# ExaScience/elprep

Measured on AMD Instinct MI355X. Metric: Mreads/s through sort+markdup+BQSR, 150bp PE, higher is better.
Workload: dtype u8/int32/int64 (integer path; float64 finalize on host)

## Files before the change

elprep_amd/csrc/adapt.hip:

```cpp
#include <cstdlib>

#include "apply_rec.hpp"
#include "common.hpp"
#include "flat.hpp"
#include "sort_plan.hpp"

namespace elp {

__global__ __launch_bounds__(256) void k_adapt_fixed(uint64_t n, const int32_t *__restrict__ pos, const int32_t *__restrict__ refid,
                                                     const uint16_t *__restrict__ flag, const uint64_t *__restrict__ cigar_off,
                                                     const uint32_t *__restrict__ cigar, int32_t *__restrict__ upos, int32_t *__restrict__ score,
                                                     uint64_t *__restrict__ key, uint32_t n_ref, int pos_bits,
                                                     const uint8_t *__restrict__ has_sr) {
  uint64_t i = (uint64_t)blockIdx.x * blockDim.x + threadIdx.x;
  if (i >= n) return;
  const uint16_t f = flag[i];
  const int32_t p = pos[i];
  const int32_t r = refid[i];
  const uint64_t ru = has_sr[i] ? (uint64_t)n_ref + 1 : (r < 0 ? (uint64_t)n_ref : (uint64_t)(uint32_t)r);
  key[i] = (ru << (pos_bits + 1)) | ((uint64_t)(uint32_t)p << 1) | ((f & F_REVERSED) ? 1ull : 0ull);
  int32_t up = 0;
  if ((f & (F_UNMAPPED | F_SECONDARY | F_SUPPLEMENTARY)) == 0) {
    const uint64_t c0 = cigar_off[i], c1 = cigar_off[i + 1];
    up = p;
    if (c1 > c0) {
      if (f & F_REVERSED) {
        int32_t clipped = 1;
        up--;
        for (uint64_t k = c1; k-- > c0;) {
          const uint32_t c = cigar[k];
          const uint32_t op = c & 0xF;
          const int32_t isclip = (op == OP_S || op == OP_H) ? 1 : 0;
          const int32_t isref = op_consumes_ref(op) ? 1 : 0;
          clipped *= isclip;
          up += (isref | clipped) * (int32_t)(c >> 4);
        }
      } else {
        for (uint64_t k = c0; k < c1; k++) {
          const uint32_t c = cigar[k];
          const uint32_t op = c & 0xF;
          if (!(op == OP_S || op == OP_H)) break;
          up -= (int32_t)(c >> 4);
        }
      }
    }
  }
  upos[i] = up;
  score[i] = 0;
}

__device__ __forceinline__ uint32_t first_bytes32(int n) { return n <= 0 ? 0u : (n >= 4 ? 0xFFFFFFFFu : (0xFFFFFFFFu >> (32 - 8 * n))); }

struct ScoreBody {
  static constexpr int NT = FL_THREADS, TILES = 4, RMAX = 1024;
  static constexpr bool TILE_ENDS = false;
  const uint16_t *__restrict__ flag;
  const uint8_t *__restrict__ qual;
  int32_t *score;
  uint64_t *qbounds;
  int32_t *acc;
  uint32_t *lo;
  uint32_t *hi;
  uint8_t *cand;
  const uint4 *mask;
  uint32_t bad;

  __device__ __forceinline__ void stage(uint32_t g0, uint32_t ng) {
    for (uint32_t k = threadIdx.x; k < ng; k += NT) {
      acc[k] = 0;
      lo[k] = 0xFFFFFFFFu;
      hi[k] = 0u;
      cand[k] = (flag[g0 + k] & (F_UNMAPPED | F_SECONDARY | F_SUPPLEMENTARY)) == 0;
    }
  }
  static __device__ __forceinline__ uint32_t part(uint32_t x, uint32_t s) {
    const uint32_t ge15 = ((x + 0x71717171u) & 0x80808080u) >> 7;
    return __builtin_amdgcn_sad_u8(x & (ge15 * 0xFFu), 0u, s);
  }
  static __device__ __forceinline__ uint32_t gt2(uint32_t x) { return (((x | 0x80808080u) - 0x03030303u) | x) & 0x80808080u; }
  static __device__ __forceinline__ uint32_t ge94(uint32_t x) { return x | (x + 0x22222222u); }
  struct Pre { Chunk ch; uint32_t rl; int nb; int k0; };
  __device__ __forceinline__ bool prefetch(uint32_t rl, int k0, int nb, uint64_t qpos, uint32_t, Pre &p) {
    p.rl = rl; p.nb = nb; p.k0 = k0;
    p.ch.load(qual + qpos);
    return true;
  }
  __device__ __forceinline__ void process(Pre &p) {
    const uint4 mk = mask[p.nb];
    const uint32_t x0 = p.ch.w0 & mk.x, x1 = p.ch.w1 & mk.y, x2 = p.ch.w2 & mk.z, x3 = p.ch.w3 & mk.w;
    const uint64_t glo = (uint64_t)gt2(x0) | ((uint64_t)gt2(x1) << 32);
    const uint64_t ghi = (uint64_t)gt2(x2) | ((uint64_t)gt2(x3) << 32);
    if (glo | ghi) {
      const int first = glo ? (__builtin_ctzll(glo) >> 3) : 8 + (__builtin_ctzll(ghi) >> 3);
      const int last = ghi ? 8 + ((63 - __builtin_clzll(ghi)) >> 3) : ((63 - __builtin_clzll(glo)) >> 3);
      atomicMin(&lo[p.rl], (uint32_t)(p.k0 + first));
      atomicMax(&hi[p.rl], (uint32_t)(p.k0 + last + 1));
    }
    if (!cand[p.rl]) return;
    bad |= (ge94(x0) | ge94(x1) | ge94(x2) | ge94(x3)) & 0x80808080u;
    const uint32_t s = part(x3, part(x2, part(x1, part(x0, 0u))));
    if (s) atomicAdd(&acc[p.rl], (int32_t)s);
  }
  __device__ __forceinline__ void group_end(uint32_t g0, uint32_t ng) {
    for (uint32_t k = threadIdx.x; k < ng; k += NT) {
      score[g0 + k] = acc[k];
      qbounds[g0 + k] = (uint64_t)hi[k] | ((uint64_t)lo[k] << 32);
    }
  }
  __device__ __forceinline__ void slots(uint32_t) {}
  __device__ __forceinline__ void retire() {}
  __device__ __forceinline__ void tile_end(uint32_t, uint64_t) {}
};

__global__ __launch_bounds__(FL_THREADS) void k_score_flat(uint64_t n, const uint64_t *__restrict__ qual_off, const uint8_t *__restrict__ qual,
                                                           uint64_t qual_bytes, const uint32_t *__restrict__ tile_first,
                                                           const uint16_t *__restrict__ flag, int32_t *score, uint64_t *qbounds, uint32_t *err) {
  __shared__ FlatLds<ScoreBody::RMAX> L;
  __shared__ int32_t acc[ScoreBody::RMAX];
  __shared__ uint32_t lo[ScoreBody::RMAX], hi[ScoreBody::RMAX];
  __shared__ uint8_t cand[ScoreBody::RMAX];
  __shared__ uint4 mask[17];
  if (threadIdx.x <= 16) {
    const int nb = (int)threadIdx.x;
    mask[nb] = make_uint4(first_bytes32(nb), first_bytes32(nb - 4), first_bytes32(nb - 8), first_bytes32(nb - 12));
  }
  __syncthreads();
  ScoreBody B{flag, qual, score, qbounds, acc, lo, hi, cand, mask, 0u};
  flat_run(qual_off, n, qual_bytes, tile_first, L, B);
  if (__any(B.bad != 0) && (threadIdx.x & 63) == 0) atomicOr(&err[0], 1u);
}

constexpr int SU_WAVES = 8, SU_MAX_LEN = 250;
__device__ __forceinline__ uint32_t su_gt2(uint32_t x) { return (((x | 0x80808080u) - 0x03030303u) | x) & 0x80808080u; }
template <int R>
__global__ __launch_bounds__(64 * SU_WAVES) void k_score_uniform(uint64_t n, uint32_t L, const uint8_t *__restrict__ qual, const uint16_t *__restrict__ flag,
                                                                 int32_t *__restrict__ score, uint64_t *__restrict__ qbounds, uint32_t *err,
                                                                 uint32_t qstride ,
                                                                 unsigned long long *qmask, const uint16_t *__restrict__ rgid, const uint16_t *__restrict__ rg_cov,
                                                                 uint2 *__restrict__ arecs ) {
  extern __shared__ __attribute__((aligned(16))) uint32_t su_lds[];
  const uint32_t lane = threadIdx.x & 63u, wave = threadIdx.x >> 6;
  const uint32_t tile_bytes = 64u * L, tile_words = tile_bytes / 4u + 4u;
  uint32_t *tile = su_lds + (size_t)wave * tile_words;
  const uint32_t s = lane * L, w0 = s >> 2, skip = s & 3u;
  const uint32_t nw = (skip + L + 3u) >> 2, tail = (skip + L) & 3u;
  const uint32_t m_first = 0xFFFFFFFFu << (8u * skip), m_last = tail ? 0xFFFFFFFFu >> (32u - 8u * tail) : 0xFFFFFFFFu;
  uint32_t bad = 0;
  uint32_t qm[3] = {0, 0, 0};
  const uint64_t ngroups = (n + 63) / 64;
  for (uint64_t g = (uint64_t)blockIdx.x * SU_WAVES + wave; g < ngroups; g += (uint64_t)gridDim.x * SU_WAVES) {
    const uint64_t r0 = g * 64;
    const uint8_t *base = qual + r0 * L;
    const uint64_t have = (n - r0 < 64 ? n - r0 : 64) * (uint64_t)L;
    uint4 v[R];
#pragma unroll
    for (int k = 0; k < R; k++) {
      const uint32_t off = (uint32_t)k * 1024u + lane * 16u;
      v[k] = make_uint4(0u, 0u, 0u, 0u);
      if (off < have) v[k] = *reinterpret_cast<const uint4 *>(base + off);
    }
#pragma unroll
    for (int k = 0; k < R; k++) {
      const uint32_t off = (uint32_t)k * 1024u + lane * 16u;
      if (off < tile_bytes) *reinterpret_cast<uint4 *>(tile + off / 4u) = v[k];
    }
    const uint64_t r = r0 + lane;
    if (r < n) {
      const uint16_t f = flag[r];
      const bool cand = (f & (F_UNMAPPED | F_SECONDARY | F_SUPPLEMENTARY)) == 0;
      const uint16_t rg = arecs ? rgid[r] : (uint16_t)ELP_NIL16;
      const uint32_t *rw = tile + w0;
      uint32_t x = rw[0] & m_first;
      if (nw == 1) x &= m_last;
      constexpr uint32_t NONE = 0xFFFFFFFFu;
      uint32_t sum = ScoreBody::part(x, 0u), orx = x;
      uint32_t kf = su_gt2(x) ? 0u : NONE, kl = 0u;
#pragma unroll 8
      for (uint32_t k = 1; k + 1 < nw; k++) {
        x = rw[k];
        sum = ScoreBody::part(x, sum);
        orx |= x;
        const bool gk = su_gt2(x) != 0u;
        kf = min(kf, gk ? k : NONE);
        kl = gk ? k : kl;
      }
      if (nw > 1) {
        x = rw[nw - 1] & m_last;
        sum = ScoreBody::part(x, sum);
        orx |= x;
        const bool gk = su_gt2(x) != 0u;
        kf = min(kf, gk ? nw - 1 : NONE);
        kl = gk ? nw - 1 : kl;
      }
      uint32_t bd = ScoreBody::ge94(orx) & 0x80808080u;
      if (bd) {
        bd = 0;
        for (uint32_t k = 0; k < nw; k++) {
          uint32_t xw = rw[k];
          if (k == 0) xw &= m_first;
          if (k == nw - 1) xw &= m_last;
          bd |= ScoreBody::ge94(xw);
        }
      }
      uint32_t lo = 0xFFFFFFFFu, hi = 0u;
      if (kf != NONE) {
        uint32_t xf = rw[kf], xl = rw[kl];
        if (kf == 0) xf &= m_first;
        if (kf == nw - 1) xf &= m_last;
        if (kl == 0) xl &= m_first;
        if (kl == nw - 1) xl &= m_last;
        lo = kf * 4u + ((uint32_t)__builtin_ctz(su_gt2(xf)) >> 3) - skip;
        hi = kl * 4u + ((31u - (uint32_t)__builtin_clz(su_gt2(xl))) >> 3) - skip + 1u;
      }
      score[r] = cand ? (int32_t)sum : 0;
      qbounds[r] = (uint64_t)hi | ((uint64_t)lo << 32);
      if (cand) bad |= bd & 0x80808080u;
      if (arecs) arecs[r] = rg == ELP_NIL16 ? make_uint2(AR_NO_RG, 0u) : apply_record(L, (int)L, f, (uint64_t)hi | ((uint64_t)lo << 32), rg_cov[rg]);
      if ((uint32_t)g % qstride == 0) {
        for (uint32_t k = 0; k < nw; k++) {
          const uint32_t vm = (k == 0 ? m_first : 0xFFFFFFFFu) & (k + 1 == nw ? m_last : 0xFFFFFFFFu), xw = rw[k];
#pragma unroll
          for (int b = 0; b < 4; b++) {
            const uint32_t q = (xw >> (8 * b)) & 0xFFu, bit = ((vm >> (8 * b)) & 1u) << (q & 31u), ws = q >> 5;
            qm[0] |= ws == 0 ? bit : 0u;
            qm[1] |= ws == 1 ? bit : 0u;
            qm[2] |= ws == 2 ? bit : 0u;
          }
        }
      }
    }
  }
  if (__any(bad != 0) && lane == 0) atomicOr(&err[0], 1u);
  if (__any((qm[0] | qm[1] | qm[2]) != 0)) {
    for (int d = 32; d >= 1; d >>= 1) {
      qm[0] |= __shfl_xor(qm[0], d, 64);
      qm[1] |= __shfl_xor(qm[1], d, 64);
      qm[2] |= __shfl_xor(qm[2], d, 64);
    }
    if (lane == 0) {
      const unsigned long long lo = (unsigned long long)qm[0] | ((unsigned long long)qm[1] << 32);
      if (lo) atomicOr(&qmask[0], lo);
      if (qm[2]) atomicOr(&qmask[1], (unsigned long long)qm[2]);
    }
  }
}
static bool score_uniform_ok(uint32_t L) {
  if (L < 16 || L > (uint32_t)SU_MAX_LEN) return false;
  if (L % 4u) return true;
  return ((L / 4u) % 4u) != 0;
}
template <int R>
static int score_uniform_launch(elp_ctx *c) {
  const uint32_t L = c->uniform_len;
  const size_t dyn = (size_t)SU_WAVES * ((size_t)64 * L + 16);
  const unsigned per_cu = (unsigned)std::max<size_t>(1, (160 * 1024) / (dyn + 256));
  const uint64_t ngroups = (c->n + 63) / 64;
  const unsigned grid = (unsigned)std::min<uint64_t>((ngroups + SU_WAVES - 1) / SU_WAVES, (uint64_t)c->n_cu * per_cu);
  ELP_HIP(c, hipFuncSetAttribute(reinterpret_cast<const void *>(&k_score_uniform<R>), hipFuncAttributeMaxDynamicSharedMemorySize, (int)dyn));
  uint2 *arecs = nullptr;
  if (L >= 16 && L <= 0x7FFF && c->n_rg > 0) {
    ELP_TRY(ensure(c, c->apply_recs, c->n + 4));
    arecs = c->apply_recs.p;
  }
  const uint32_t qstride = (uint32_t)std::min<uint64_t>(128, std::max<uint64_t>(1, ngroups / 8192));
  ELP_LAUNCH(c, "adapt_score", k_score_uniform<R>, dim3(grid), dim3(64 * SU_WAVES), dyn, c->n, L, (const uint8_t *)c->qual.p, (const uint16_t *)c->flag.p,
             c->score.p, c->qbounds.p, c->adapt_err.p, qstride, reinterpret_cast<unsigned long long *>(c->adapt_err.p + 2), (const uint16_t *)c->rgid.p,
             (const uint16_t *)c->rg_cov.p, arecs);
  c->derived.adapt_sampled = true;
  c->derived.apply_recs_valid = arecs != nullptr;
  c->apply_recs_lmax = (int)L;
  return 0;
}
static int score_uniform(elp_ctx *c) {
  switch ((c->uniform_len + 15u) / 16u) {
#define ELP_SU(R) case R: return score_uniform_launch<R>(c);
    ELP_SU(1) ELP_SU(2) ELP_SU(3) ELP_SU(4) ELP_SU(5) ELP_SU(6) ELP_SU(7) ELP_SU(8) ELP_SU(9) ELP_SU(10) ELP_SU(11) ELP_SU(12) ELP_SU(13) ELP_SU(14)
    ELP_SU(15) ELP_SU(16)
#undef ELP_SU
  }
  return set_error(c, ELP_ERR_ARG, "score_uniform: read length %u", c->uniform_len);
}

__global__ __launch_bounds__(256) void k_qual_present_sample(const uint8_t *__restrict__ qual, uint64_t qual_bytes, uint64_t stride, uint64_t span,
                                                             unsigned long long *qmask) {
  const uint64_t ntiles = (qual_bytes + FL_TILE - 1) / FL_TILE;
  uint32_t m[3] = {0, 0, 0};
  for (uint64_t t = (uint64_t)blockIdx.x * stride; t < ntiles; t += (uint64_t)gridDim.x * stride) {
    const uint64_t tb = t * FL_TILE, te = (tb + span < qual_bytes) ? tb + span : qual_bytes;
    for (uint64_t p = tb + (uint64_t)threadIdx.x * 16; p < te; p += 256 * 16) {
      Chunk ch;
      ch.load(qual + p);
      const int nv = (int)((te - p) < 16 ? (te - p) : 16);
#pragma unroll
      for (int i = 0; i < 16; i++) {
        const uint32_t wv = (i >> 2) == 0 ? ch.w0 : ((i >> 2) == 1 ? ch.w1 : ((i >> 2) == 2 ? ch.w2 : ch.w3));
        const uint32_t q = (wv >> (8 * (i & 3))) & 0xFFu;
        const uint32_t bit = (i < nv) ? (1u << (q & 31u)) : 0u;
        const uint32_t wsel = q >> 5;
        m[0] |= wsel == 0 ? bit : 0u;
        m[1] |= wsel == 1 ? bit : 0u;
        m[2] |= wsel == 2 ? bit : 0u;
      }
    }
  }
  for (int d = 32; d >= 1; d >>= 1) {
    m[0] |= __shfl_xor(m[0], d, 64);
    m[1] |= __shfl_xor(m[1], d, 64);
    m[2] |= __shfl_xor(m[2], d, 64);
  }
  if ((threadIdx.x & 63) == 0) {
    const unsigned long long lo = (unsigned long long)m[0] | ((unsigned long long)m[1] << 32);
    if (lo) atomicOr(&qmask[0], lo);
    if (m[2]) atomicOr(&qmask[1], (unsigned long long)m[2]);
  }
}

__global__ __launch_bounds__(256) void k_flat_index(const uint64_t *__restrict__ qual_off, uint64_t n_reads, uint64_t ntiles,
                                                    uint32_t *__restrict__ tile_first) {
  const uint64_t t = (uint64_t)blockIdx.x * blockDim.x + threadIdx.x;
  if (t > ntiles) return;
  if (t == ntiles) { tile_first[t] = (uint32_t)n_reads; return; }
  const uint64_t x = t * FL_TILE;
  uint64_t lo = 0, hi = n_reads;
  while (lo < hi) {
    const uint64_t mid = lo + (hi - lo) / 2;
    if (qual_off[mid] >= x) hi = mid; else lo = mid + 1;
  }
  tile_first[t] = (uint32_t)lo;
}

int ensure_flat_index(elp_ctx *c) {
  if (c->derived.has_flat_index(c->n, c->qual_bytes)) return 0;
  const uint64_t ntiles = (c->qual_bytes + FL_TILE - 1) / FL_TILE;
  ELP_TRY(ensure(c, c->tile_first, ntiles + 2));
  if (c->n)
    ELP_LAUNCH(c, "flat_index", k_flat_index, dim3(blocks_for(ntiles + 1, 256)), dim3(256), 0, (const uint64_t *)c->qual_off.p, c->n, ntiles,
               c->tile_first.p);
  c->derived.flat_index_n = c->n;
  c->derived.flat_index_bytes = c->qual_bytes;
  return 0;
}

__global__ __launch_bounds__(256) void k_uniform_check(uint64_t n, const uint64_t *__restrict__ qual_off, const uint64_t *__restrict__ seq_off,
                                                       const uint32_t *__restrict__ l_seq, uint64_t len, uint64_t sb, uint64_t seq_front, uint32_t *bad) {
  const uint64_t i = (uint64_t)blockIdx.x * blockDim.x + threadIdx.x;
  bool b = false;
  if (i < n) b = qual_off[i] != i * len || seq_off[i] != seq_front + i * sb || (uint64_t)l_seq[i] != len;
  if (i == n) b = qual_off[n] != n * len || seq_off[n] != seq_front + n * sb;
  if (__any(b) && (threadIdx.x & 63) == 0) atomicOr(bad, 1u);
}
int ensure_uniform_len(elp_ctx *c) {
  if (c->derived.has_uniform(c->n, c->qual_bytes)) return 0;
  c->uniform_len = 0;
  c->derived.uniform_n = c->n;
  c->derived.uniform_bytes = c->qual_bytes;
  if (!c->n || c->qual_bytes % c->n) return 0;
  const uint64_t len = c->qual_bytes / c->n;
  if (len == 0 || len > 0x3FFFFFull) return 0;
  uint32_t *bad = c->err_flag.p + 2;
  ELP_HIP(c, hipMemsetAsync(bad, 0, 4, c->stream));
  ELP_LAUNCH(c, "uniform_check", k_uniform_check, dim3(blocks_for(c->n + 1, 256)), dim3(256), 0, c->n, (const uint64_t *)c->qual_off.p,
             (const uint64_t *)c->seq_off.p, (const uint32_t *)c->l_seq.p, len, (len + 1) / 2, (uint64_t)elp_ctx::SEQ_FRONT, bad);
  uint32_t hb = 0;
  ELP_HIP(c, hipMemcpyAsync(&hb, bad, 4, hipMemcpyDeviceToHost, c->stream));
  ELP_HIP(c, elp::stream_wait(c->stream));
  ELP_HIP(c, hipMemsetAsync(bad, 0, 4, c->stream));
  if (!hb) c->uniform_len = (uint32_t)len;
  return 0;
}

int adapt_quality_error(elp_ctx *c) {
  return set_error(c, ELP_ERR_DATA, "Invalid QUAL character (phred > 93) in a duplicate-marking candidate (reference: log.Panic, filters/mark-duplicates.go:64-66)");
}

static int adapt_resolve(elp_ctx *c) {
  if (!c->derived.adapt_pending) return 0;
  uint32_t w[ADAPT_WORDS];
  ELP_HIP(c, hipMemcpyAsync(w, c->adapt_err.p, sizeof w, hipMemcpyDeviceToHost, c->stream));
  ELP_HIP(c, elp::stream_wait(c->stream));
  adapt_note(c, w);
  return 0;
}
void adapt_note(elp_ctx *c, const uint32_t *words) {
  c->derived.adapt_word_read((words[0] & 1u) != 0);
  if (c->derived.adapt_sampled) {
    c->adapt_qmask[0] = (unsigned long long)words[2] | ((unsigned long long)words[3] << 32);
    c->adapt_qmask[1] = (unsigned long long)words[4] | ((unsigned long long)words[5] << 32);
  }
}
int adapt_begin(elp_ctx *c, int *pos_bits_out) {
  ELP_HIP(c, hipSetDevice(c->device));
  const uint64_t n = c->n;
  ELP_TRY(ensure_flat_index(c));
  ELP_TRY(ensure(c, c->upos, n + 1));
  ELP_TRY(ensure(c, c->score, n + 1));
  ELP_TRY(ensure(c, c->key, n + 1));
  ELP_TRY(ensure(c, c->qbounds, n + 1));
  ELP_TRY(ensure(c, c->adapt_err, ADAPT_WORDS + 2));
  ELP_HIP(c, hipMemsetAsync(c->adapt_err.p, 0, ADAPT_WORDS * sizeof(uint32_t), c->stream));
  c->derived.adapt_begins();
  const KeyWidth kw = key_width(c->max_pos, c->n_ref);
  c->key_bits = kw.key_bits;
  *pos_bits_out = kw.pos_bits;
  return 0;
}
int adapt_scores(elp_ctx *c) {
  const uint64_t n = c->n;
  if (!n) return 0;
  if (!c->qual_bytes) {
    ELP_HIP(c, hipMemsetAsync(c->qbounds.p, 0, n * sizeof(uint64_t), c->stream));
    ELP_HIP(c, hipMemsetAsync(c->score.p, 0, n * sizeof(int32_t), c->stream));
    return 0;
  }
  ELP_TRY(ensure_uniform_len(c));
  if (c->uniform_len && score_uniform_ok(c->uniform_len) && c->tune.score_kernel != 1) {
    ELP_TRY(score_uniform(c));
  } else {
    ELP_HIP(c, hipMemsetAsync(c->score.p, 0, n * sizeof(int32_t), c->stream));
    const unsigned grid = (unsigned)std::min<uint64_t>(flat_steps<ScoreBody>(c->qual_bytes), (uint64_t)c->n_cu * 4);
    ELP_LAUNCH(c, "adapt_score_flat", k_score_flat, dim3(grid), dim3(FL_THREADS), 0, n, (const uint64_t *)c->qual_off.p, (const uint8_t *)c->qual.p,
               c->qual_bytes, (const uint32_t *)c->tile_first.p, (const uint16_t *)c->flag.p, c->score.p, c->qbounds.p, c->adapt_err.p);
  }
  c->derived.adapt_pending = true;
  return 0;
}
int ensure_adapted(elp_ctx *c, bool check_quals) {
  if (c->derived.adapted()) {
    if (check_quals) ELP_TRY(adapt_resolve(c));
    return (check_quals && c->derived.adapt_bad_qual) ? adapt_quality_error(c) : 0;
  }
  int pos_bits = 1;
  ELP_TRY(adapt_begin(c, &pos_bits));
  const uint64_t n = c->n;
  if (n) {
    ELP_LAUNCH(c, "adapt_fixed", k_adapt_fixed, dim3(blocks_for(n, 256)), dim3(256), 0, n, (const int32_t *)c->pos.p, (const int32_t *)c->refid.p,
               (const uint16_t *)c->flag.p, (const uint64_t *)c->cigar_off.p, (const uint32_t *)c->cigar.p, c->upos.p, c->score.p, c->key.p,
               (uint32_t)c->n_ref, pos_bits, (const uint8_t *)c->has_sr.p);
    ELP_TRY(adapt_scores(c));
  }
  c->derived.keys = c->derived.scores = true;
  if (check_quals) ELP_TRY(adapt_resolve(c));
  return (check_quals && c->derived.adapt_bad_qual) ? adapt_quality_error(c) : 0;
}
int ensure_keys(elp_ctx *c) { return c->derived.keys ? 0 : ensure_adapted(c, false); }

int ensure_qual_present(elp_ctx *c, bool exact) {
  if (c->derived.have_qual_present) return 0;
  c->qual_present[0] = c->qual_present[1] = 0;
  if (!exact && c->tune.qual_hint != 1 && c->derived.scores && c->derived.adapt_sampled) {
    ELP_TRY(adapt_resolve(c));
    c->qual_present[0] = c->adapt_qmask[0];
    c->qual_present[1] = c->adapt_qmask[1];
  } else if (c->qual_bytes && (exact || c->tune.qual_hint != 1)) {
    unsigned long long *qm;
    ELP_TRY(scratch(c, 6, 4, &qm));
    ELP_HIP(c, hipMemsetAsync(qm, 0, 16, c->stream));
    const uint64_t ntiles = (c->qual_bytes + FL_TILE - 1) / FL_TILE;
    const uint64_t stride = exact ? 1 : std::min<uint64_t>(16, std::max<uint64_t>(1, ntiles / 2048));
    const unsigned grid = (unsigned)std::min<uint64_t>((ntiles + stride - 1) / stride, 2048);
    ELP_LAUNCH(c, "qual_present_sample", k_qual_present_sample, dim3(grid), dim3(256), 0, (const uint8_t *)c->qual.p, c->qual_bytes, stride,
               (exact || stride == 1) ? FL_TILE : (uint64_t)4096, qm);
    ELP_HIP(c, hipMemcpyAsync(c->qual_present, qm, 16, hipMemcpyDeviceToHost, c->stream));
    ELP_HIP(c, elp::stream_wait(c->stream));
  }
  if (!exact && c->tune.qual_hint_drop >= 0) {
    const int q = c->tune.qual_hint_drop;
    if (q < 64) c->qual_present[0] &= ~(1ull << q);
    else if (q < 128) c->qual_present[1] &= ~(1ull << (q - 64));
  }
  c->derived.have_qual_present = true;
  return 0;
}

}
```

elprep_amd/csrc/common.hpp:

```cpp
#pragma once

#include <hip/hip_runtime.h>

#include <sched.h>

#include <cstdarg>
#include <cstdint>
#include <cstdio>
#include <cstring>
#include <map>
#include <mutex>
#include <string>
#include <vector>

#include "../../include/elprep_hip.h"
#include "../../include/elprep_hip_debug.h"
#include "apply_plan.hpp"
#include "derived.hpp"

namespace elp {

constexpr int WAVE = 64;

enum : uint16_t {
  F_MULTIPLE = 0x1, F_PROPER = 0x2, F_UNMAPPED = 0x4, F_NEXT_UNMAPPED = 0x8, F_REVERSED = 0x10, F_NEXT_REVERSED = 0x20,
  F_FIRST = 0x40, F_LAST = 0x80, F_SECONDARY = 0x100, F_QCFAILED = 0x200, F_DUPLICATE = 0x400, F_SUPPLEMENTARY = 0x800
};

enum : uint32_t { OP_M = 0, OP_I = 1, OP_D = 2, OP_N = 3, OP_S = 4, OP_H = 5, OP_P = 6, OP_EQ = 7, OP_X = 8 };

__host__ __device__ inline bool op_consumes_read(uint32_t op) { return op == OP_M || op == OP_I || op == OP_S || op == OP_EQ || op == OP_X; }
__host__ __device__ inline bool op_consumes_ref(uint32_t op) { return op == OP_M || op == OP_D || op == OP_N || op == OP_EQ || op == OP_X; }

size_t debug_guard_bytes();
void debug_guard_arm(void *p, size_t payload_bytes);
void debug_guard_release(void *p);
int debug_guard_check_all();

template <class T>
struct DVec {
  T *p = nullptr;
  size_t cap = 0;
  DVec() = default;
  DVec(const DVec &) = delete;
  DVec &operator=(const DVec &) = delete;
  ~DVec() { release(); }
  void release() {
    if (p) { debug_guard_release(p); (void)hipFree(p); }
    p = nullptr;
    cap = 0;
  }
  size_t bytes() const { return cap * sizeof(T); }
};

struct ProfPending {
  int name_id;
  hipEvent_t a, b;
};

}

struct elp_ctx {
  int device = 0;
  int n_cu = 256;
  hipStream_t stream = nullptr;
  std::string err;
  std::mutex stage_mu;

  bool have_header = false;
  int32_t n_ref = 0, n_rg = 0, n_lib = 0, n_cov = 0;
  std::vector<int32_t> h_ref_len;
  std::vector<uint16_t> h_rg_lib, h_rg_cov;
  elp::DVec<int32_t> ref_len;
  elp::DVec<uint16_t> rg_lib, rg_cov;
  bool dict_replaced = false;
  int32_t n_ref0 = 0;
  std::vector<int32_t> h_ref_len0;

  static constexpr uint64_t SEQ_FRONT = 16;
  uint64_t n = 0, qname_bytes = 0, cigar_ops = 0, seq_bytes = SEQ_FRONT, qual_bytes = 0;
  uint64_t n_sr = 0;
  uint64_t n_filtered = 0;
  elp::DVec<int32_t> refid, pos, next_refid, pnext, tlen;
  elp::DVec<uint16_t> flag, rgid, split;
  elp::DVec<uint8_t> mapq, has_sr;
  elp::DVec<uint32_t> l_seq;
  elp::DVec<uint64_t> qname_off, cigar_off, seq_off, qual_off;
  elp::DVec<uint8_t> qname, seq4, qual;
  elp::DVec<uint32_t> cigar;
  elp::DVec<uint64_t> stage_tmp;
  uint32_t max_qname_len = 0, max_l_seq = 0;
  uint32_t max_split = 0;
  uint32_t max_pos = 0;
  int key_bits = 64;

  elp::Derived derived;
  bool radix_check_pending = false;
  elp::DVec<uint32_t> adapt_err;
  unsigned long long adapt_qmask[2] = {0, 0};
  elp::DVec<uint2> apply_recs;
  int apply_recs_lmax = 0;
  unsigned long long qual_present[2] = {0, 0};
  elp::DVec<int32_t> upos, score;
  elp::DVec<uint64_t> qbounds;
  elp::DVec<uint64_t> key;
  elp::DVec<uint32_t> perm;
  elp::DVec<uint32_t> err_flag;
  elp::DVec<uint32_t> tile_first;
  void *h_pinned = nullptr;
  size_t h_pinned_cap = 0;
  elp::DVec<unsigned long long> radix_state;
  elp::DVec<uint32_t> radix_ticket;
  elp::DVec<unsigned long long> radix_hist;
  elp::DVec<uint32_t> scan_pool;
  elp::DVec<unsigned long long> xchg_hdr;
  elp::DVec<uint32_t> tie_live;
  elp::DVec<uint32_t> md_ctr;
  static constexpr uint32_t MAX_QNAME = 1000;
  static constexpr uint32_t TIE_LIVE_WORDS = 32;
  uint32_t radix_epoch = 0;
  uint32_t uniform_len = 0;

  elp::DVec<uint32_t> mate;
  elp::DVec<uint32_t> pair_win;

  std::vector<uint8_t *> h_ref_seq;
  std::vector<int64_t> h_ref_seq_len;
  std::vector<int32_t *> h_sites;
  std::vector<int64_t> h_n_sites;
  std::vector<uint8_t> ref_flags_dirty;
  std::vector<uint32_t *> h_site_idx;
  elp::DVec<uint8_t *> d_ref_seq;
  elp::DVec<int64_t> d_ref_seq_len;
  elp::DVec<int32_t *> d_sites;
  elp::DVec<uint32_t *> d_site_idx;
  elp::DVec<int64_t> d_n_sites;
  bool bqsr_ptrs_dirty = true;

  static constexpr size_t TABLES_TAIL = 4096;
  elp::DVec<unsigned long long> dev_tables;
  size_t tables_n = 0;
  int tables_max_cycle = 0;
  unsigned long long tables_quals[2] = {0, 0};
  elp::DVec<unsigned long long> tables_pack;
  elp::DVec<uint8_t> lut_rows_dev;
  void *comm = nullptr;
  bool comm_borrowed = false;
  int (*xport)(void *, int64_t *, size_t) = nullptr;
  void *xport_user = nullptr;
  int (*p2p)(void *, int, const void *, size_t, int, void *, size_t) = nullptr;
  void *p2p_user = nullptr;
  int group_rank = 0, group_world = 1;
  elp_ctx *group_owner = nullptr;
  std::vector<elp_ctx *> group_borrowers;

  elp::DVec<uint8_t> raw;
  elp::DVec<uint64_t> raw_off;
  uint64_t raw_n = 0, raw_bytes = 0;
  uint64_t max_raw_rec = 0;
  elp::DVec<uint8_t> rg_ids;
  elp::DVec<uint32_t> rg_ids_off;
  bool have_rg_ids = false;
  elp::DVec<uint8_t> ref_names;
  elp::DVec<uint32_t> ref_names_off;
  std::string h_ref_names;
  std::vector<uint32_t> h_ref_names_off;
  uint32_t max_ref_name = 0;
  bool have_ref_names = false;
  elp::DVec<uint32_t> ref_name_slots;
  uint32_t ref_name_mask = 0;
  bool have_ref_name_table = false;
  static constexpr size_t TAG_WORDS = 65536 / 32;
  bool tag_filter = false;
  std::vector<uint32_t> h_tag_drop;
  elp::DVec<uint32_t> tag_drop;
  bool replace_rg = false;
  std::string replace_rg_id;
  elp::DVec<uint8_t> replace_rg_dev;
  hipStream_t copy_stream = nullptr;
  elp::DVec<uint8_t> lut_dev;
  void *lut_pinned = nullptr;
  size_t lut_pinned_cap = 0;
  hipEvent_t lut_ev = nullptr;
  hipEvent_t apply_ev = nullptr;
  int lut_uploaded_cycle = 0;
  elp::DVec<uint32_t> lut_wk;
  elp::LutDictBuilt dict_built;
  hipEvent_t tables_ev = nullptr;
  void *bounce[2] = {nullptr, nullptr};
  hipEvent_t bounce_ev[2] = {nullptr, nullptr};

  uint32_t *mail = nullptr;
  hipEvent_t mail_ev = nullptr;

  elp_ctx *side[2] = {nullptr, nullptr};
  hipEvent_t side_ev[2] = {nullptr, nullptr};
  hipEvent_t side_done[2] = {nullptr, nullptr};
  bool sort_ahead = false;
  uint64_t presort_n = 0;
  uint64_t *presort_ks = nullptr;
  int presort_idx_bits = 0;

  elp::DVec<uint16_t> snap_flag;
  elp::DVec<uint8_t> snap_qual;
  uint64_t snap_n = 0, snap_qual_bytes = 0;

  struct Tuning {
    int count_kernel = 0;
    int apply_kernel = 0;
    int count3_rlog = -1;
    int qual_hint = 0;
    int qual_hint_drop = -1;
    int pair_table_slots = 1 << 20;
    long long bgzf_piece = 1ll << 30;
    int bgzf_weak_guess = 0;
    int score_kernel = 0;
    int mate_path = 0;
    int radix_tile = 0;
    int sort_pairs = 0;
    int tie_rounds = 0;
    int exchange_piece = 0;
    int emit_pass = 0;
    int sam_pass = 0;
    long long bgzf_inflate_piece = 2ll << 30;
    int bgzf_copy_chunk = 0;
    int bgzf_tok_lds = 0;
    int bgzf_first_chunk_div = 4;
    int bgzf_fixed = 0;
    int bgzf_tok_fail_above = 0;
    int bgzf_stored = 0;
    int apply_wgs = 0;
    int count3_grid = 0;
    int presort_tile = 0;
    int side_priority = 0;
  } tune;

  elp::DVec<uint8_t> scratch[8];

  bool profiling = false;
  const char *prof_prefix = nullptr;
  std::vector<std::string> prof_names;
  std::map<std::string, int> prof_index;
  std::vector<uint64_t> prof_launches;
  std::vector<double> prof_ms;
  std::vector<elp::ProfPending> prof_pending;
};

namespace elp {

class LaneViews {
  struct Item { void *vec; void (*take_back)(void *); };
  std::vector<Item> items;

 public:
  template <class... Col>
  LaneViews(elp_ctx *shadow, elp_ctx *ctx, Col... cols) { (view(shadow->*cols, ctx->*cols), ...); }
  LaneViews(const LaneViews &) = delete;
  LaneViews &operator=(const LaneViews &) = delete;
  ~LaneViews() {
    for (const Item &it : items) it.take_back(it.vec);
  }
  template <class T>
  void view(DVec<T> &to, const DVec<T> &from, bool with_cap = false) {
    to.p = from.p;
    to.cap = with_cap ? from.cap : 0;
    items.push_back(Item{&to, [](void *v) { DVec<T> *d = static_cast<DVec<T> *>(v); d->p = nullptr; d->cap = 0; }});
  }
};

int set_error(elp_ctx *c, int code, const char *fmt, ...);
int prof_begin(elp_ctx *c, const char *name);
void prof_end(elp_ctx *c, int pending);
int prof_flush(elp_ctx *c);
struct ProfScope {
  elp_ctx *c;
  const char *saved;
  ProfScope(elp_ctx *ctx, const char *prefix) : c(ctx), saved(ctx->prof_prefix) { ctx->prof_prefix = prefix; }
  ~ProfScope() { c->prof_prefix = saved; }
};

#define ELP_HIP(ctx, call)                                                                             \
  do {                                                                                                 \
    hipError_t e__ = (call);                                                                           \
    if (e__ != hipSuccess)                                                                             \
      return elp::set_error((ctx), e__ == hipErrorOutOfMemory ? ELP_ERR_NOMEM : ELP_ERR_HIP, "%s failed: %s (%s:%d)", #call, \
                            hipGetErrorString(e__), __FILE__, __LINE__);                               \
  } while (0)

#define ELP_TRY(expr)            \
  do {                           \
    int rc__ = (expr);           \
    if (rc__ != 0) return rc__;  \
  } while (0)

bool sync_spin();
inline void spin_relax(unsigned &spins) {
  if (++spins < 4096u) {
#if defined(__x86_64__) || defined(__i386__)
    __builtin_ia32_pause();
#elif defined(__aarch64__)
    asm volatile("yield");
#endif
  } else {
    sched_yield();
  }
}
inline hipError_t stream_wait(hipStream_t st) {
  if (!sync_spin()) return hipStreamSynchronize(st);
  hipError_t e;
  unsigned spins = 0;
  while ((e = hipStreamQuery(st)) == hipErrorNotReady) spin_relax(spins);
  return e;
}
inline hipError_t event_wait(hipEvent_t ev) {
  if (!sync_spin()) return hipEventSynchronize(ev);
  hipError_t e;
  unsigned spins = 0;
  while ((e = hipEventQuery(ev)) == hipErrorNotReady) spin_relax(spins);
  return e;
}

int debug_poison();
bool debug_trace();

template <class T>
int ensure(elp_ctx *c, DVec<T> &v, size_t n, bool keep = false, size_t keep_elems = 0) {
  if (n <= v.cap) return 0;
  size_t ncap = keep ? (n + n / 2 + 16) : n;
  T *np = nullptr;
  ELP_HIP(c, hipMalloc((void **)&np, ncap * sizeof(T) + debug_guard_bytes()));
  if (debug_guard_bytes()) debug_guard_arm(np, ncap * sizeof(T));
  if (const int pz = debug_poison(); pz >= 0) {
    ELP_HIP(c, hipMemsetAsync(np, pz, ncap * sizeof(T), c->stream));
    ELP_HIP(c, elp::stream_wait(c->stream));
  }
  if (keep && v.p && keep_elems) {
    hipError_t e = hipMemcpyAsync(np, v.p, keep_elems * sizeof(T), hipMemcpyDeviceToDevice, c->stream);
    if (e == hipSuccess) e = elp::stream_wait(c->stream);
    if (e != hipSuccess) {
      (void)hipFree(np);
      return set_error(c, ELP_ERR_HIP, "device copy failed while growing a column: %s", hipGetErrorString(e));
    }
  }
  if (v.p) {
    (void)elp::stream_wait(c->stream);
    debug_guard_release(v.p);
    if (debug_poison() >= 0) { (void)hipMemsetAsync(v.p, 0xDD, v.cap * sizeof(T), c->stream); (void)elp::stream_wait(c->stream); }
    (void)hipFree(v.p);
  }
  v.p = np;
  v.cap = ncap;
  return 0;
}

template <class T>
int scratch(elp_ctx *c, int slot, size_t n, T **out) {
  ELP_TRY(ensure(c, c->scratch[slot], n * sizeof(T) + 256));
  *out = reinterpret_cast<T *>(c->scratch[slot].p);
  return 0;
}

#define ELP_LAUNCH(ctx, name, kernel, grid, block, shmem, ...)                              \
  do {                                                                                      \
    int pp__ = (ctx)->profiling ? elp::prof_begin((ctx), (name)) : -1;                      \
    if (elp::debug_trace()) fprintf(stderr, "[elp] %s\n", (name));                          \
    hipLaunchKernelGGL(kernel, grid, block, shmem, (ctx)->stream, __VA_ARGS__);             \
    if (pp__ >= 0) elp::prof_end((ctx), pp__);                                              \
    ELP_HIP((ctx), hipGetLastError());                                                      \
    if (elp::debug_trace()) ELP_HIP((ctx), elp::stream_wait((ctx)->stream));            \
  } while (0)

inline unsigned blocks_for(uint64_t n, unsigned per_block) { return (unsigned)((n + per_block - 1) / per_block); }

__device__ __forceinline__ uint64_t mix64(uint64_t x) {
  x ^= x >> 30; x *= 0xbf58476d1ce4e5b9ull; x ^= x >> 27; x *= 0x94d049bb133111ebull; x ^= x >> 31;
  return x;
}

__device__ __forceinline__ uint64_t load8(const uint8_t *__restrict__ p) {
  uint64_t w;
  __builtin_memcpy(&w, p, 8);
  return w;
}
__device__ __forceinline__ uint64_t low_bytes(uint64_t w, uint32_t nbytes) {
  return nbytes >= 8 ? w : (w & ((1ull << (8 * nbytes)) - 1ull));
}
__device__ inline int qname_cmp(const uint8_t *__restrict__ q, const uint64_t *__restrict__ off, uint32_t a, uint32_t b) {
  const uint64_t oa = off[a], ob = off[b];
  const uint32_t la = (uint32_t)(off[a + 1] - oa), lb = (uint32_t)(off[b + 1] - ob);
  const uint32_t m = la < lb ? la : lb;
  for (uint32_t i = 0; i < m; i += 8) {
    const uint32_t nb = m - i;
    const uint64_t wa = low_bytes(load8(q + oa + i), nb), wb = low_bytes(load8(q + ob + i), nb);
    if (wa != wb) {
      const uint64_t ba = __builtin_bswap64(wa), bb = __builtin_bswap64(wb);
      return ba < bb ? -1 : 1;
    }
  }
  return la < lb ? -1 : (la > lb ? 1 : 0);
}
__device__ inline bool qname_eq(const uint8_t *__restrict__ q, const uint64_t *__restrict__ off, uint32_t a, uint32_t b) {
  const uint64_t oa = off[a], ob = off[b];
  const uint32_t la = (uint32_t)(off[a + 1] - oa), lb = (uint32_t)(off[b + 1] - ob);
  if (la != lb) return false;
  uint64_t diff = 0;
  for (uint32_t i = 0; i < la && diff == 0; i += 32) {
    const uint64_t a0 = load8(q + oa + i), a1 = load8(q + oa + i + 8), a2 = load8(q + oa + i + 16), a3 = load8(q + oa + i + 24);
    const uint64_t b0 = load8(q + ob + i), b1 = load8(q + ob + i + 8), b2 = load8(q + ob + i + 16), b3 = load8(q + ob + i + 24);
    const uint32_t nb = la - i;
    diff |= low_bytes(a0 ^ b0, nb);
    diff |= nb > 8 ? low_bytes(a1 ^ b1, nb - 8) : 0ull;
    diff |= nb > 16 ? low_bytes(a2 ^ b2, nb - 16) : 0ull;
    diff |= nb > 24 ? low_bytes(a3 ^ b3, nb - 24) : 0ull;
  }
  return diff == 0;
}

__host__ __device__ inline uint16_t mod_flag(uint16_t flag) {
  if ((flag & F_MULTIPLE) == 0) flag &= (uint16_t) ~(F_NEXT_UNMAPPED | F_NEXT_REVERSED);
  if (flag & F_UNMAPPED) flag &= (uint16_t)~F_REVERSED;
  if (flag & F_NEXT_UNMAPPED) flag &= (uint16_t)~F_NEXT_REVERSED;
  return flag;
}

inline void commit_rejects(elp_ctx *c, unsigned long long dropped, unsigned long long tagged) {
  c->n_sr += dropped;
  c->n_filtered += dropped + tagged;
}

int radix_sort_pairs(elp_ctx *c, uint64_t *keys, uint32_t *vals, uint64_t *keys_tmp, uint32_t *vals_tmp, uint64_t n,
                     uint64_t **keys_out, uint32_t **vals_out);
int radix_sort_fused(elp_ctx *c, const uint64_t *keycol, uint64_t n, int key_bits, int idx_bits, uint64_t *buf0, uint64_t *buf1, uint64_t **out);
struct RadixBounds {
  uint32_t *start = nullptr, *nend = nullptr;
  uint32_t mask = 0;
  int shift = 0;
};
int radix_sort_pairs_low(elp_ctx *c, uint64_t *keys, uint32_t *vals, uint64_t *keys_tmp, uint32_t *vals_tmp, uint64_t n, int ndigits,
                         uint64_t **keys_out, uint32_t **vals_out, const uint64_t *first_src = nullptr, bool identity_vals = false,
                         const uint32_t *n_dev = nullptr , RadixBounds bnd = RadixBounds{});
int exclusive_scan_u32(elp_ctx *c, const uint32_t *in, uint32_t *out, uint64_t n, uint32_t *total_host );
int ensure_adapted(elp_ctx *c, bool check_quals = true);
int ensure_keys(elp_ctx *c);
int adapt_begin(elp_ctx *c, int *pos_bits);
int adapt_scores(elp_ctx *c);
int mailbox(elp_ctx *c);
int side_lane(elp_ctx *c, int lane, elp_ctx **out);
int side_join(elp_ctx *c, int lane);
int sort_presort(elp_ctx *c);
void prof_merge_side(elp_ctx *c);
constexpr int ADAPT_WORDS = 6;
void adapt_note(elp_ctx *c, const uint32_t *words );
int adapt_quality_error(elp_ctx *c);
int ensure_uniform_len(elp_ctx *c);
int ensure_qual_present(elp_ctx *c, bool exact = false);
int fetch_err(elp_ctx *c, uint32_t *words );
int radix_check(elp_ctx *c);
void group_release(elp_ctx *c);
int group_sendrecv(elp_ctx *c, int send_peer, const void *send_dev, size_t send_bytes, int recv_peer, void *recv_dev, size_t recv_bytes);
int tables_written(elp_ctx *c);
int stage_reserve(elp_ctx *c, uint64_t n, uint64_t qb, uint64_t co, uint64_t sb, uint64_t lb);
constexpr uint32_t MERGE_SECOND = 0x80000000u;
int keep_concat_src(elp_ctx *groups, uint64_t ng, uint64_t ns, uint32_t *g0_dev, uint32_t *src);
int merge_refuses_queryname(elp_ctx *groups, const char *who);
int merge_spread_slots(elp_ctx *groups, elp_ctx *spread, uint64_t **slots_out);
int keep_coordinate_order(elp_ctx *c, uint64_t n_out, uint64_t *keys, uint32_t *bad_dev, bool *in_order);
int stage_recode_seq(elp_ctx *c, uint64_t from, uint64_t bytes);
inline void clear_run_settings(elp_ctx *c) { c->tag_filter = false; c->replace_rg = false; c->replace_rg_id.clear(); }
inline bool same_replace_rg(const elp_ctx *a, const elp_ctx *b) { return a->replace_rg == b->replace_rg && a->replace_rg_id == b->replace_rg_id; }
int install_dictionary(elp_ctx *c, int32_t n_ref, const int32_t *ref_len);
int staging_refused_after_replace(elp_ctx *c, const char *who);
int stage_bam_columns(elp_ctx *c, uint32_t n_rec, uint64_t piece_bytes, uint64_t raw_end, uint64_t max_raw_rec, uint16_t split_id);
int bgzf_frame(elp_ctx *c, const uint8_t *raw, uint64_t n_bytes, uint8_t *out);
int bgzf_deflate(elp_ctx *c, const uint8_t *raw, uint64_t n_bytes, uint8_t *out, uint64_t *out_bytes);

}
```

elprep_amd/csrc/ctx.hip:

```cpp
#include "common.hpp"

namespace elp {

namespace {
constexpr size_t GUARD = 4096;
constexpr uint8_t GUARD_BYTE = 0xC3;
std::mutex guard_mu;
std::map<void *, size_t> guard_of;
int guard_check_one(void *p, size_t payload) {
  uint8_t host[GUARD];
  if (hipDeviceSynchronize() != hipSuccess || hipMemcpy(host, static_cast<uint8_t *>(p) + payload, GUARD, hipMemcpyDeviceToHost) != hipSuccess) return 0;
  for (size_t k = 0; k < GUARD; k++)
    if (host[k] != GUARD_BYTE) {
      fprintf(stderr, "[elp] ELP_DEBUG_GUARD: byte %zu behind the end of a %zu-byte device buffer was overwritten (0x%02x)\n", k, payload, host[k]);
      return 1;
    }
  return 0;
}
}
size_t debug_guard_bytes() {
  static const size_t v = [] { const char *e = getenv("ELP_DEBUG_GUARD"); return (e && *e && *e != '0') ? GUARD : (size_t)0; }();
  return v;
}
void debug_guard_arm(void *p, size_t payload) {
  (void)hipMemset(static_cast<uint8_t *>(p) + payload, GUARD_BYTE, GUARD);
  (void)hipDeviceSynchronize();
  std::lock_guard<std::mutex> lk(guard_mu);
  guard_of[p] = payload;
}
void debug_guard_release(void *p) {
  if (!debug_guard_bytes()) return;
  size_t payload = 0;
  {
    std::lock_guard<std::mutex> lk(guard_mu);
    auto it = guard_of.find(p);
    if (it == guard_of.end()) return;
    payload = it->second;
    guard_of.erase(it);
  }
  if (guard_check_one(p, payload)) abort();
}
int debug_guard_check_all() {
  if (!debug_guard_bytes()) return 0;
  std::lock_guard<std::mutex> lk(guard_mu);
  int bad = 0;
  for (auto &kv : guard_of) bad += guard_check_one(kv.first, kv.second);
  return bad;
}

bool sync_spin() {
  static const bool v = [] { const char *e = getenv("ELP_SYNC_SPIN"); return !(e && *e == '0'); }();
  return v;
}
bool debug_trace() {
  static const bool v = [] { const char *e = getenv("ELP_DEBUG_TRACE"); return e && *e && *e != '0'; }();
  return v;
}
int debug_poison() {
  static const int v = [] {
    const char *e = getenv("ELP_DEBUG_POISON");
    return (e && *e) ? (int)(strtol(e, nullptr, 0) & 0xFF) : -1;
  }();
  return v;
}


int set_error(elp_ctx *c, int code, const char *fmt, ...) {
  char buf[1024];
  va_list ap;
  va_start(ap, fmt);
  vsnprintf(buf, sizeof buf, fmt, ap);
  va_end(ap);
  if (c) c->err = buf;
  return code;
}

int prof_begin(elp_ctx *c, const char *name0) {
  const std::string name = c->prof_prefix ? std::string(c->prof_prefix) + name0 : std::string(name0);
  auto it = c->prof_index.find(name);
  int id;
  if (it == c->prof_index.end()) {
    id = (int)c->prof_names.size();
    c->prof_names.push_back(name);
    c->prof_index[name] = id;
    c->prof_launches.push_back(0);
    c->prof_ms.push_back(0.0);
  } else {
    id = it->second;
  }
  ProfPending p;
  p.name_id = id;
  if (hipEventCreate(&p.a) != hipSuccess) return -1;
  if (hipEventCreate(&p.b) != hipSuccess) { (void)hipEventDestroy(p.a); return -1; }
  (void)hipEventRecord(p.a, c->stream);
  c->prof_pending.push_back(p);
  return (int)c->prof_pending.size() - 1;
}
void prof_end(elp_ctx *c, int pending) { (void)hipEventRecord(c->prof_pending[pending].b, c->stream); }
int prof_flush(elp_ctx *c) {
  if (c->prof_pending.empty()) return 0;
  ELP_HIP(c, elp::stream_wait(c->stream));
  for (auto &p : c->prof_pending) {
    float ms = 0.f;
    if (hipEventElapsedTime(&ms, p.a, p.b) == hipSuccess) {
      c->prof_ms[p.name_id] += ms;
      c->prof_launches[p.name_id] += 1;
    }
    (void)hipEventDestroy(p.a);
    (void)hipEventDestroy(p.b);
  }
  c->prof_pending.clear();
  return 0;
}

__global__ void k_rebase_offsets(const uint64_t *__restrict__ src, uint64_t *__restrict__ dst, uint64_t n_plus_1, uint64_t base,
                                 uint64_t src0) {
  uint64_t i = (uint64_t)blockIdx.x * blockDim.x + threadIdx.x;
  if (i < n_plus_1) dst[i] = src[i] - src0 + base;
}

__device__ __forceinline__ uint32_t recode_byte(uint32_t b) {
  constexpr uint64_t TAB = 0x8888888388828108ull;
  return (uint32_t)((TAB >> (4 * (b >> 4))) & 15u) | ((uint32_t)((TAB >> (4 * (b & 15u))) & 15u) << 4);
}
__global__ __launch_bounds__(256) void k_recode_seq(uint8_t *__restrict__ seq, uint64_t nbytes) {
  const uint64_t i = ((uint64_t)blockIdx.x * blockDim.x + threadIdx.x) * 16;
  if (i >= nbytes) return;
  if (i + 16 <= nbytes) {
    uint32_t w[4];
    __builtin_memcpy(w, seq + i, 16);
#pragma unroll
    for (int k = 0; k < 4; k++) {
      const uint32_t x = w[k];
      w[k] = recode_byte(x & 0xFFu) | (recode_byte((x >> 8) & 0xFFu) << 8) | (recode_byte((x >> 16) & 0xFFu) << 16) | (recode_byte(x >> 24) << 24);
    }
    __builtin_memcpy(seq + i, w, 16);
  } else {
    for (uint64_t k = i; k < nbytes; k++) seq[k] = (uint8_t)recode_byte(seq[k]);
  }
}

int stage_recode_seq(elp_ctx *c, uint64_t from, uint64_t bytes) {
  hipLaunchKernelGGL(k_recode_seq, dim3(blocks_for((bytes + 15) / 16, 256)), dim3(256), 0, c->stream, c->seq4.p + from, bytes);
  ELP_HIP(c, hipGetLastError());
  return 0;
}

int fetch_err(elp_ctx *c, uint32_t *words) {
  ELP_HIP(c, hipMemcpyAsync(words, c->err_flag.p, 4 * sizeof(uint32_t), hipMemcpyDeviceToHost, c->stream));
  ELP_HIP(c, elp::stream_wait(c->stream));
  c->radix_check_pending = false;
  if (words[0] & 256u) {
    const uint32_t w0 = words[0] & ~256u;
    ELP_HIP(c, hipMemcpyAsync(c->err_flag.p, &w0, 4, hipMemcpyHostToDevice, c->stream));
    ELP_HIP(c, elp::stream_wait(c->stream));
    c->derived.radix_timed_out();
    return set_error(c, ELP_ERR_HIP, "radix sort: tile look-back timed out");
  }
  return 0;
}
int mailbox(elp_ctx *c) {
  if (!c->mail) ELP_HIP(c, hipHostMalloc((void **)&c->mail, 1024 * sizeof(uint32_t), hipHostMallocDefault));
  if (!c->mail_ev) ELP_HIP(c, hipEventCreateWithFlags(&c->mail_ev, hipEventDisableTiming));
  return 0;
}
int side_lane(elp_ctx *c, int lane, elp_ctx **out) {
  if (!c->side[lane]) {
    elp_ctx *s = new elp_ctx();
    s->device = c->device;
    s->n_cu = c->n_cu;
    int prio_lo = 0, prio_hi = 0;
    (void)hipDeviceGetStreamPriorityRange(&prio_lo, &prio_hi);
    const hipError_t se = c->tune.side_priority != 1 ? hipStreamCreateWithFlags(&s->stream, hipStreamNonBlocking)
                                                     : hipStreamCreateWithPriority(&s->stream, hipStreamNonBlocking, prio_hi);
    if (se != hipSuccess || ensure(s, s->err_flag, 4) != 0 ||
        hipMemsetAsync(s->err_flag.p, 0, 16, s->stream) != hipSuccess) {
      if (s->stream) (void)hipStreamDestroy(s->stream);
      delete s;
      return set_error(c, ELP_ERR_HIP, "the side lane's stream could not be made");
    }
    c->side[lane] = s;
  }
  if (!c->side_ev[lane]) ELP_HIP(c, hipEventCreateWithFlags(&c->side_ev[lane], hipEventDisableTiming));
  if (!c->side_done[lane]) ELP_HIP(c, hipEventCreateWithFlags(&c->side_done[lane], hipEventDisableTiming));
  ELP_HIP(c, hipEventRecord(c->side_ev[lane], c->stream));
  ELP_HIP(c, hipStreamWaitEvent(c->side[lane]->stream, c->side_ev[lane], 0));
  c->side[lane]->profiling = c->profiling;
  c->side[lane]->tune = c->tune;
  *out = c->side[lane];
  return 0;
}
int side_join(elp_ctx *c, int lane) {
  ELP_HIP(c, hipEventRecord(c->side_done[lane], c->side[lane]->stream));
  ELP_HIP(c, hipStreamWaitEvent(c->stream, c->side_done[lane], 0));
  return 0;
}
void prof_merge_side(elp_ctx *c) {
  for (int lane = 0; lane < 2; lane++) {
    elp_ctx *s = c->side[lane];
    if (!s) continue;
    (void)prof_flush(s);
    for (size_t k = 0; k < s->prof_names.size(); k++) {
      if (!s->prof_launches[k]) continue;
      auto it = c->prof_index.find(s->prof_names[k]);
      int id;
      if (it == c->prof_index.end()) {
        id = (int)c->prof_names.size();
        c->prof_names.push_back(s->prof_names[k]);
        c->prof_index[s->prof_names[k]] = id;
        c->prof_launches.push_back(0);
        c->prof_ms.push_back(0.0);
      } else {
        id = it->second;
      }
      c->prof_launches[id] += s->prof_launches[k];
      c->prof_ms[id] += s->prof_ms[k];
      s->prof_launches[k] = 0;
      s->prof_ms[k] = 0.0;
    }
  }
}
int radix_check(elp_ctx *c) {
  if (!c->radix_check_pending) return 0;
  uint32_t e[4];
  return fetch_err(c, e);
}

int release_bqsr_inputs(elp_ctx *c) {
  ELP_HIP(c, elp::stream_wait(c->stream));
  for (auto &p : c->h_ref_seq) if (p) { (void)hipFree(p); p = nullptr; }
  for (auto &p : c->h_sites) if (p) { (void)hipFree(p); p = nullptr; }
  for (auto &p : c->h_site_idx) if (p) { (void)hipFree(p); p = nullptr; }
  for (auto &v : c->h_ref_seq_len) v = 0;
  for (auto &v : c->h_n_sites) v = 0;
  c->bqsr_ptrs_dirty = true;
  return 0;
}
int install_dictionary(elp_ctx *c, int32_t n_ref, const int32_t *ref_len) {
  ELP_TRY(ensure(c, c->ref_len, (size_t)n_ref + 1));
  ELP_TRY(release_bqsr_inputs(c));
  const std::vector<int32_t> len(ref_len, ref_len + n_ref);
  c->n_ref = n_ref;
  c->h_ref_len = len;
  c->have_ref_names = false;
  c->have_ref_name_table = false;
  if (n_ref) ELP_HIP(c, hipMemcpyAsync(c->ref_len.p, c->h_ref_len.data(), (size_t)n_ref * sizeof(int32_t), hipMemcpyHostToDevice, c->stream));
  ELP_HIP(c, elp::stream_wait(c->stream));
  c->h_ref_seq.assign((size_t)n_ref, nullptr);
  c->h_ref_seq_len.assign((size_t)n_ref, 0);
  c->h_sites.assign((size_t)n_ref, nullptr);
  c->h_site_idx.assign((size_t)n_ref, nullptr);
  c->h_n_sites.assign((size_t)n_ref, 0);
  c->ref_flags_dirty.assign((size_t)n_ref, 0);
  c->bqsr_ptrs_dirty = true;
  return 0;
}
int staging_refused_after_replace(elp_ctx *c, const char *who) {
  return set_error(c, ELP_ERR_ARG, "%s: the reference dictionary was replaced (elp_replace_reference_dictionary): the staged refids are the new "
                   "dictionary's, the header's are the old one's; call elp_reset or elp_set_header first", who);
}

}

using namespace elp;

extern "C" {

int elp_debug_check_guards(void) { return elp::debug_guard_check_all(); }


int elp_create(int device_ordinal, elp_ctx **out) {
  if (!out) return ELP_ERR_ARG;
  *out = nullptr;
  int ndev = 0;
  if (hipGetDeviceCount(&ndev) != hipSuccess || ndev <= 0) return ELP_ERR_HIP;
  if (device_ordinal < 0 || device_ordinal >= ndev) return ELP_ERR_ARG;
  if (hipSetDevice(device_ordinal) != hipSuccess) return ELP_ERR_HIP;
  hipDeviceProp_t prop;
  if (hipGetDeviceProperties(&prop, device_ordinal) != hipSuccess) return ELP_ERR_HIP;
  if (strncmp(prop.gcnArchName, "gfx950", 6) != 0) return ELP_ERR_UNSUPPORTED;
  elp_ctx *c = new elp_ctx();
  c->device = device_ordinal;
  c->n_cu = prop.multiProcessorCount > 0 ? prop.multiProcessorCount : 256;
  if (hipStreamCreateWithFlags(&c->stream, hipStreamNonBlocking) != hipSuccess) { delete c; return ELP_ERR_HIP; }
  if (ensure(c, c->err_flag, 4) != 0 || hipMemsetAsync(c->err_flag.p, 0, 16, c->stream) != hipSuccess) { delete c; return ELP_ERR_HIP; }
  *out = c;
  return ELP_OK;
}

void elp_destroy(elp_ctx *c) {
  if (!c) return;
  (void)hipSetDevice(c->device);
  (void)elp::stream_wait(c->stream);
  for (auto &p : c->prof_pending) { (void)hipEventDestroy(p.a); (void)hipEventDestroy(p.b); }
  if (c->lut_pinned) (void)hipHostFree(c->lut_pinned);
  if (c->lut_ev) (void)hipEventDestroy(c->lut_ev);
  if (c->apply_ev) (void)hipEventDestroy(c->apply_ev);
  for (auto p : c->h_ref_seq) if (p) (void)hipFree(p);
  for (auto p : c->h_sites) if (p) (void)hipFree(p);
  for (auto p : c->h_site_idx) if (p) (void)hipFree(p);
  if (c->h_pinned) (void)hipHostFree(c->h_pinned);
  for (int lane = 0; lane < 2; lane++) {
    if (c->side[lane]) {
      (void)elp::stream_wait(c->side[lane]->stream);
      for (auto &p : c->side[lane]->prof_pending) { (void)hipEventDestroy(p.a); (void)hipEventDestroy(p.b); }
      (void)hipStreamDestroy(c->side[lane]->stream);
      delete c->side[lane];
      c->side[lane] = nullptr;
    }
    if (c->side_ev[lane]) (void)hipEventDestroy(c->side_ev[lane]);
    if (c->side_done[lane]) (void)hipEventDestroy(c->side_done[lane]);
  }
  if (c->mail) (void)hipHostFree(c->mail);
  if (c->mail_ev) (void)hipEventDestroy(c->mail_ev);
  for (int k = 0; k < 2; k++) {
    if (c->bounce[k]) (void)hipHostFree(c->bounce[k]);
    if (c->bounce_ev[k]) (void)hipEventDestroy(c->bounce_ev[k]);
  }
  if (c->copy_stream) (void)hipStreamDestroy(c->copy_stream);
  if (c->tables_ev) (void)hipEventDestroy(c->tables_ev);
  group_release(c);
  (void)hipStreamDestroy(c->stream);
  delete c;
}

const char *elp_last_error(const elp_ctx *c) { return c ? c->err.c_str() : "null context"; }

int elp_sync(elp_ctx *c) {
  if (!c) return ELP_ERR_ARG;
  if (c->radix_check_pending) return radix_check(c);
  ELP_HIP(c, elp::stream_wait(c->stream));
  return 0;
}

void *elp_stream(elp_ctx *c) { return c ? (void *)c->stream : nullptr; }

int elp_set_header(elp_ctx *c, const elp_header *h) {
  if (!c || !h || h->n_ref < 0 || h->n_rg < 0 || (h->n_ref && !h->ref_len) || (h->n_rg && (!h->rg_lib || !h->rg_cov)))
    return set_error(c, ELP_ERR_ARG, "elp_set_header: bad arguments");
  ELP_HIP(c, hipSetDevice(c->device));
  if (c->dict_replaced) ELP_TRY(release_bqsr_inputs(c));
  c->n_ref = h->n_ref; c->n_rg = h->n_rg; c->n_lib = h->n_lib; c->n_cov = h->n_cov;
  c->derived.header_changed();
  clear_run_settings(c);
  c->h_ref_len.assign(h->ref_len, h->ref_len + h->n_ref);
  c->n_ref0 = h->n_ref;
  c->h_ref_len0 = c->h_ref_len;
  c->dict_replaced = false;
  c->have_ref_names = false;
  c->have_ref_name_table = false;
  c->h_rg_lib.assign(h->rg_lib, h->rg_lib + h->n_rg);
  c->h_rg_cov.assign(h->rg_cov, h->rg_cov + h->n_rg);
  for (int i = 0; i < h->n_rg; i++) {
    if (c->h_rg_lib[i] != ELP_NIL16 && c->h_rg_lib[i] >= h->n_lib) return set_error(c, ELP_ERR_ARG, "rg_lib[%d] out of range", i);
    if (c->h_rg_cov[i] >= h->n_cov) return set_error(c, ELP_ERR_ARG, "rg_cov[%d] out of range", i);
  }
  ELP_TRY(ensure(c, c->ref_len, (size_t)h->n_ref + 1));
  ELP_TRY(ensure(c, c->rg_lib, (size_t)h->n_rg + 1));
  ELP_TRY(ensure(c, c->rg_cov, (size_t)h->n_rg + 1));
  if (h->n_ref) ELP_HIP(c, hipMemcpyAsync(c->ref_len.p, h->ref_len, h->n_ref * sizeof(int32_t), hipMemcpyHostToDevice, c->stream));
  if (h->n_rg) {
    ELP_HIP(c, hipMemcpyAsync(c->rg_lib.p, h->rg_lib, h->n_rg * sizeof(uint16_t), hipMemcpyHostToDevice, c->stream));
    ELP_HIP(c, hipMemcpyAsync(c->rg_cov.p, h->rg_cov, h->n_rg * sizeof(uint16_t), hipMemcpyHostToDevice, c->stream));
  }
  ELP_HIP(c, elp::stream_wait(c->stream));
  c->h_ref_seq.resize(h->n_ref, nullptr);
  c->h_ref_seq_len.resize(h->n_ref, 0);
  c->h_sites.resize(h->n_ref, nullptr);
  c->h_site_idx.resize(h->n_ref, nullptr);
  c->h_n_sites.resize(h->n_ref, 0);
  c->ref_flags_dirty.assign(h->n_ref, 0);
  c->bqsr_ptrs_dirty = true;
  c->have_header = true;
  return 0;
}

}
namespace elp {
int stage_reserve(elp_ctx *c, uint64_t n, uint64_t qb, uint64_t co, uint64_t sb, uint64_t lb) {
  bool keep = c->n > 0;
  ELP_TRY(ensure(c, c->refid, n, keep, c->n));
  ELP_TRY(ensure(c, c->pos, n, keep, c->n));
  ELP_TRY(ensure(c, c->next_refid, n, keep, c->n));
  ELP_TRY(ensure(c, c->pnext, n, keep, c->n));
  ELP_TRY(ensure(c, c->tlen, n, keep, c->n));
  ELP_TRY(ensure(c, c->flag, n, keep, c->n));
  ELP_TRY(ensure(c, c->rgid, n, keep, c->n));
  ELP_TRY(ensure(c, c->split, n, keep, c->n));
  ELP_TRY(ensure(c, c->mapq, n, keep, c->n));
  ELP_TRY(ensure(c, c->has_sr, n, keep, c->n));
  ELP_TRY(ensure(c, c->l_seq, n, keep, c->n));
  ELP_TRY(ensure(c, c->qname_off, n + 1, keep, c->n + 1));
  ELP_TRY(ensure(c, c->cigar_off, n + 1, keep, c->n + 1));
  ELP_TRY(ensure(c, c->seq_off, n + 1, keep, c->n + 1));
  ELP_TRY(ensure(c, c->qual_off, n + 1, keep, c->n + 1));
  ELP_TRY(ensure(c, c->qname, qb + 64, keep, c->qname_bytes));
  ELP_TRY(ensure(c, c->cigar, co + 4, keep, c->cigar_ops));
  ELP_TRY(ensure(c, c->seq4, sb + 32, keep, c->seq_bytes));
  ELP_TRY(ensure(c, c->qual, lb + 32, keep, c->qual_bytes));
  return 0;
}
}
extern "C" {

int elp_reserve(elp_ctx *c, uint64_t n, uint64_t qb, uint64_t co, uint64_t sb, uint64_t lb) {
  if (!c) return ELP_ERR_ARG;
  std::lock_guard<std::mutex> g(c->stage_mu);
  ELP_HIP(c, hipSetDevice(c->device));
  return stage_reserve(c, n, qb, co, sb + elp_ctx::SEQ_FRONT, lb);
}

int elp_reset(elp_ctx *c) {
  if (!c) return ELP_ERR_ARG;
  std::lock_guard<std::mutex> g(c->stage_mu);
  c->n = c->qname_bytes = c->cigar_ops = c->qual_bytes = 0;
  c->seq_bytes = elp_ctx::SEQ_FRONT;
  c->n_sr = 0;
  c->n_filtered = 0;
  c->raw_n = c->raw_bytes = 0;
  c->max_raw_rec = 0;
  c->max_split = 0;
  c->max_qname_len = c->max_l_seq = 0;
  c->max_pos = 0;
  c->derived.records_changed();
  clear_run_settings(c);
  if (c->dict_replaced) {
    ELP_HIP(c, hipSetDevice(c->device));
    ELP_TRY(install_dictionary(c, c->n_ref0, c->h_ref_len0.data()));
    c->derived.header_changed();
    c->dict_replaced = false;
  }
  return 0;
}

uint64_t elp_num_records(const elp_ctx *c) { return c ? c->n : 0; }
uint64_t elp_num_sorted(const elp_ctx *c) { return c ? c->n - c->n_sr : 0; }
uint64_t elp_num_qual_bytes(const elp_ctx *c) { return c ? c->qual_bytes : 0; }

int elp_stage(elp_ctx *c, const elp_batch *b) {
  if (!c || !b) return ELP_ERR_ARG;
  std::lock_guard<std::mutex> g(c->stage_mu);
  ELP_HIP(c, hipSetDevice(c->device));
  if (!c->have_header) return set_error(c, ELP_ERR_ARG, "elp_stage: call elp_set_header first");
  if (c->dict_replaced) return staging_refused_after_replace(c, "elp_stage");
  uint64_t n = b->n;
  if (n == 0) return 0;
  if (c->n + n > 0xFFFFFFF0ull) return set_error(c, ELP_ERR_UNSUPPORTED, "more than 2^32-16 records per context");
  uint64_t q0 = b->qname_off[0], c0 = b->cigar_off[0], s0 = b->seq_off[0], l0 = b->qual_off[0];
  uint64_t qb = b->qname_off[n] - q0, co = b->cigar_off[n] - c0, sb = b->seq_off[n] - s0, lb = b->qual_off[n] - l0;
  ELP_TRY(stage_reserve(c, c->n + n, c->qname_bytes + qb, c->cigar_ops + co, c->seq_bytes + sb, c->qual_bytes + lb));
  hipStream_t st = c->stream;
  uint64_t at = c->n;
#define H2D(dst, src, cnt, T) ELP_HIP(c, hipMemcpyAsync((dst), (src), (cnt) * sizeof(T), hipMemcpyHostToDevice, st))
  if (lb) H2D(c->qual.p + c->qual_bytes, b->qual + l0, lb, uint8_t);
  if (sb) {
    H2D(c->seq4.p + c->seq_bytes, b->seq4 + s0, sb, uint8_t);
    hipLaunchKernelGGL(k_recode_seq, dim3(blocks_for((sb + 15) / 16, 256)), dim3(256), 0, st, c->seq4.p + c->seq_bytes, sb);
    ELP_HIP(c, hipGetLastError());
  }
  if (qb) H2D(c->qname.p + c->qname_bytes, b->qname + q0, qb, uint8_t);
  if (co) H2D(c->cigar.p + c->cigar_ops, b->cigar + c0, co, uint32_t);
  H2D(c->refid.p + at, b->refid, n, int32_t);
  H2D(c->pos.p + at, b->pos, n, int32_t);
  H2D(c->next_refid.p + at, b->next_refid, n, int32_t);
  H2D(c->pnext.p + at, b->pnext, n, int32_t);
  H2D(c->tlen.p + at, b->tlen, n, int32_t);
  H2D(c->flag.p + at, b->flag, n, uint16_t);
  H2D(c->rgid.p + at, b->rgid, n, uint16_t);
  if (b->split) H2D(c->split.p + at, b->split, n, uint16_t);
  else ELP_HIP(c, hipMemsetAsync(c->split.p + at, 0, n * sizeof(uint16_t), st));
  H2D(c->mapq.p + at, b->mapq, n, uint8_t);
  H2D(c->l_seq.p + at, b->l_seq, n, uint32_t);
  if (b->has_sr) H2D(c->has_sr.p + at, b->has_sr, n, uint8_t);
  else ELP_HIP(c, hipMemsetAsync(c->has_sr.p + at, 0, n, st));
  ELP_TRY(ensure(c, c->stage_tmp, 4 * (n + 1)));
  unsigned blk = 256, grd = blocks_for(n + 1, blk);
  struct { const uint64_t *src; uint64_t *dst; uint64_t base; } offs[4] = {
      {b->qname_off, c->qname_off.p + at, c->qname_bytes}, {b->cigar_off, c->cigar_off.p + at, c->cigar_ops},
      {b->seq_off, c->seq_off.p + at, c->seq_bytes}, {b->qual_off, c->qual_off.p + at, c->qual_bytes}};
  for (int k = 0; k < 4; k++) H2D(c->stage_tmp.p + (size_t)k * (n + 1), offs[k].src, n + 1, uint64_t);
  for (int k = 0; k < 4; k++) {
    hipLaunchKernelGGL(k_rebase_offsets, dim3(grd), dim3(blk), 0, st, (const uint64_t *)(c->stage_tmp.p + (size_t)k * (n + 1)), offs[k].dst, n + 1, offs[k].base,
                       offs[k].src[0]);
    ELP_HIP(c, hipGetLastError());
  }
#undef H2D
  uint64_t n_sr = 0;
  uint32_t max_split = c->max_split;
  uint32_t max_qname_len = c->max_qname_len, max_l_seq = c->max_l_seq, max_pos = c->max_pos;
  int scan_rc = 0;
  for (uint64_t i = 0; i < n && !scan_rc; i++) {
    uint64_t ql = b->qname_off[i + 1] - b->qname_off[i];
    if (ql > elp_ctx::MAX_QNAME) scan_rc = set_error(c, ELP_ERR_UNSUPPORTED, "record %llu: QNAME of %llu bytes (limit %u)", (unsigned long long)i, (unsigned long long)ql, elp_ctx::MAX_QNAME);
    if (b->has_sr && b->has_sr[i]) n_sr++;
    if (b->split && b->split[i] > max_split) max_split = b->split[i];
    if (ql > max_qname_len) max_qname_len = (uint32_t)ql;
    if (b->l_seq[i] > max_l_seq) max_l_seq = b->l_seq[i];
    if ((uint32_t)b->pos[i] > max_pos) max_pos = (uint32_t)b->pos[i];
    if (b->qual_off[i + 1] - b->qual_off[i] > 0x3FFFFFull || b->l_seq[i] > 0x3FFFFFu)
      scan_rc = set_error(c, ELP_ERR_UNSUPPORTED, "record %llu: more than 4194303 bases", (unsigned long long)i);
    if (b->rgid[i] != ELP_NIL16 && b->rgid[i] >= c->n_rg) scan_rc = set_error(c, ELP_ERR_ARG, "record %llu: rgid %u not in header", (unsigned long long)i, b->rgid[i]);
    if (b->refid[i] >= c->n_ref) scan_rc = set_error(c, ELP_ERR_ARG, "record %llu: refid %d not in header", (unsigned long long)i, b->refid[i]);
  }
  if (scan_rc) { (void)elp::stream_wait(st); return scan_rc; }
  ELP_HIP(c, elp::stream_wait(st));
  c->n += n; c->qname_bytes += qb; c->cigar_ops += co; c->seq_bytes += sb; c->qual_bytes += lb;
  c->n_sr += n_sr;
  c->max_split = max_split;
  c->max_qname_len = max_qname_len; c->max_l_seq = max_l_seq; c->max_pos = max_pos;
  c->derived.records_changed();
  return 0;
}

int elp_stage_columns(elp_ctx *c, uint64_t n, const int32_t *refid, const int32_t *pos, const int32_t *next_refid, const int32_t *pnext, const int32_t *tlen,
                      const uint16_t *flag, const uint8_t *mapq, const uint16_t *rgid, const uint8_t *has_sr, const uint32_t *l_seq,
                      const uint64_t *qname_off, const uint8_t *qname, const uint64_t *cigar_off, const uint32_t *cigar, const uint64_t *seq_off,
                      const uint8_t *seq4, const uint64_t *qual_off, const uint8_t *qual, const uint16_t *split) {
  if (!c) return ELP_ERR_ARG;
  if (n && (!refid || !pos || !next_refid || !pnext || !tlen || !flag || !mapq || !rgid || !l_seq || !qname_off || !cigar_off || !seq_off || !qual_off))
    return set_error(c, ELP_ERR_ARG, "elp_stage_columns: a required column is NULL");
  elp_batch b;
  b.n = n; b.refid = refid; b.pos = pos; b.next_refid = next_refid; b.pnext = pnext; b.tlen = tlen; b.flag = flag; b.mapq = mapq; b.rgid = rgid;
  b.has_sr = has_sr; b.l_seq = l_seq; b.qname_off = qname_off; b.qname = qname; b.cigar_off = cigar_off; b.cigar = cigar; b.seq_off = seq_off;
  b.seq4 = seq4; b.qual_off = qual_off; b.qual = qual; b.split = split;
  return elp_stage(c, &b);
}

int elp_set_header_columns(elp_ctx *c, int32_t n_ref, const int32_t *ref_len, int32_t n_rg, const uint16_t *rg_lib, const uint16_t *rg_cov, int32_t n_lib,
                           int32_t n_cov) {
  elp_header h;
  h.n_ref = n_ref; h.ref_len = ref_len; h.n_rg = n_rg; h.rg_lib = rg_lib; h.rg_cov = rg_cov; h.n_lib = n_lib; h.n_cov = n_cov;
  return elp_set_header(c, &h);
}

static int d2h(elp_ctx *c, void *dst, const void *src, size_t bytes) {
  if (!bytes) return 0;
  ELP_HIP(c, hipSetDevice(c->device));
  ELP_HIP(c, hipMemcpyAsync(dst, src, bytes, hipMemcpyDeviceToHost, c->stream));
  ELP_HIP(c, elp::stream_wait(c->stream));
  return 0;
}

int elp_get_permutation(elp_ctx *c, uint32_t *out) {
  if (!c || (!out && c->n)) return ELP_ERR_ARG;
  if (!c->derived.sorted) return set_error(c, ELP_ERR_ARG, "elp_get_permutation: call elp_sort_coordinate, elp_sort_queryname or elp_order_keep first");
  ELP_TRY(radix_check(c));
  return d2h(c, out, c->perm.p, c->n * sizeof(uint32_t));
}
int elp_get_flags(elp_ctx *c, uint16_t *out) {
  if (!c || (!out && c->n)) return ELP_ERR_ARG;
  ELP_TRY(radix_check(c));
  return d2h(c, out, c->flag.p, c->n * sizeof(uint16_t));
}
int elp_get_adapted(elp_ctx *c, int32_t *upos, int32_t *score) {
  if (!c) return ELP_ERR_ARG;
  ELP_TRY(ensure_adapted(c));
  if (upos) ELP_TRY(d2h(c, upos, c->upos.p, c->n * sizeof(int32_t)));
  if (score) ELP_TRY(d2h(c, score, c->score.p, c->n * sizeof(int32_t)));
  return 0;
}
int elp_get_qual(elp_ctx *c, uint8_t *out) {
  if (!c || (!out && c->qual_bytes)) return ELP_ERR_ARG;
  return d2h(c, out, c->qual.p, c->qual_bytes);
}

int elp_snapshot(elp_ctx *c) {
  if (!c) return ELP_ERR_ARG;
  ELP_HIP(c, hipSetDevice(c->device));
  ELP_TRY(ensure(c, c->snap_flag, c->n + 1));
  ELP_TRY(ensure(c, c->snap_qual, c->qual_bytes + 16));
  if (c->n) ELP_HIP(c, hipMemcpyAsync(c->snap_flag.p, c->flag.p, c->n * sizeof(uint16_t), hipMemcpyDeviceToDevice, c->stream));
  if (c->qual_bytes) ELP_HIP(c, hipMemcpyAsync(c->snap_qual.p, c->qual.p, c->qual_bytes, hipMemcpyDeviceToDevice, c->stream));
  c->snap_n = c->n;
  c->snap_qual_bytes = c->qual_bytes;
  c->derived.have_snapshot = true;
  return 0;
}
int elp_rollback(elp_ctx *c) {
  if (!c) return ELP_ERR_ARG;
  if (!c->derived.have_snapshot || c->snap_n != c->n || c->snap_qual_bytes != c->qual_bytes)
    return set_error(c, ELP_ERR_ARG, "elp_rollback: no snapshot of the current record set");
  ELP_HIP(c, hipSetDevice(c->device));
  if (c->n) ELP_HIP(c, hipMemcpyAsync(c->flag.p, c->snap_flag.p, c->n * sizeof(uint16_t), hipMemcpyDeviceToDevice, c->stream));
  if (c->qual_bytes) ELP_HIP(c, hipMemcpyAsync(c->qual.p, c->snap_qual.p, c->qual_bytes, hipMemcpyDeviceToDevice, c->stream));
  c->derived.flag_qual_restored();
  return 0;
}

int elp_set_tuning(elp_ctx *c, const char *key, int64_t value) {
  if (!c || !key) return ELP_ERR_ARG;
  const std::string k(key);
  const int v = (int)value;
  if (k == "count_kernel") c->tune.count_kernel = v;
  else if (k == "apply_kernel") c->tune.apply_kernel = v;
  else if (k == "bgzf_piece") { if (value < 1) return set_error(c, ELP_ERR_ARG, "elp_set_tuning: bgzf_piece must be positive"); c->tune.bgzf_piece = value; }
  else if (k == "bgzf_weak_guess") c->tune.bgzf_weak_guess = v;
  else if (k == "score_kernel") { c->tune.score_kernel = v; c->derived.score_tuning_changed(); }
  else if (k == "count3_rlog") c->tune.count3_rlog = v;
  else if (k == "qual_hint") { c->tune.qual_hint = v; c->derived.hint_tuning_changed(); }
  else if (k == "qual_hint_drop") { c->tune.qual_hint_drop = v; c->derived.hint_tuning_changed(); }
  else if (k == "pair_table_slots") {
    if (v == 0) { c->tune.pair_table_slots = 1 << 20; return 0; }
    if (v < 2 || v > (1 << 20) || (v & (v - 1))) return set_error(c, ELP_ERR_ARG, "elp_set_tuning: pair_table_slots must be a power of two >= 2");
    c->tune.pair_table_slots = v;
  } else if (k == "mate_path") {
    if (value != 0 && value != 2) return set_error(c, ELP_ERR_ARG, "elp_set_tuning: mate_path is 0 (the library decides) or 2 (every candidate through the table)");
    c->tune.mate_path = v;
  } else if (k == "tie_rounds") c->tune.tie_rounds = v;
  else if (k == "radix_tile") c->tune.radix_tile = v;
  else if (k == "sort_pairs") c->tune.sort_pairs = v;
  else if (k == "exchange_piece") c->tune.exchange_piece = v;
  else if (k == "emit_pass") c->tune.emit_pass = v;
  else if (k == "sam_pass") c->tune.sam_pass = v;
  else if (k == "bgzf_stored") c->tune.bgzf_stored = v;
  else if (k == "bgzf_tok_fail_above") c->tune.bgzf_tok_fail_above = v;
  else if (k == "bgzf_fixed") c->tune.bgzf_fixed = v;
  else if (k == "bgzf_first_chunk_div") c->tune.bgzf_first_chunk_div = v;
  else if (k == "bgzf_tok_lds") c->tune.bgzf_tok_lds = v;
  else if (k == "bgzf_copy_chunk") c->tune.bgzf_copy_chunk = v;
  else if (k == "bgzf_inflate_piece") { if (value < 1) return set_error(c, ELP_ERR_ARG, "elp_set_tuning: bgzf_inflate_piece must be positive"); c->tune.bgzf_inflate_piece = value; }
  else if (k == "md_fused" || k == "bgzf_inflate") {
    if (value != 0) return set_error(c, ELP_ERR_ARG, "elp_set_tuning: key '%s' is retired (only 0 is accepted)", key);
  } else if (k == "apply_wgs") c->tune.apply_wgs = v;
  else if (k == "presort_tile") c->tune.presort_tile = v;
  else if (k == "count3_grid") { if (value < 0) return set_error(c, ELP_ERR_ARG, "elp_set_tuning: count3_grid must not be negative"); c->tune.count3_grid = v; }
  else if (k == "side_priority") c->tune.side_priority = v;
  else return set_error(c, ELP_ERR_ARG, "elp_set_tuning: unknown key '%s'", key);
  return 0;
}

int elp_profile_enable(elp_ctx *c, int on) {
  if (!c) return ELP_ERR_ARG;
  if (!on) { ELP_TRY(prof_flush(c)); prof_merge_side(c); }
  c->profiling = on != 0;
  for (int lane = 0; lane < 2; lane++)
    if (c->side[lane]) c->side[lane]->profiling = c->profiling;
  return 0;
}
int elp_profile_reset(elp_ctx *c) {
  if (!c) return ELP_ERR_ARG;
  ELP_TRY(prof_flush(c));
  prof_merge_side(c);
  for (auto &v : c->prof_launches) v = 0;
  for (auto &v : c->prof_ms) v = 0.0;
  return 0;
}
int elp_profile_count(elp_ctx *c) {
  if (!c) return ELP_ERR_ARG;
  if (prof_flush(c) != 0) return ELP_ERR_HIP;
  prof_merge_side(c);
  return (int)c->prof_names.size();
}
int elp_profile_get(elp_ctx *c, int index, const char **name, uint64_t *launches, double *total_ms) {
  if (!c || index < 0 || index >= (int)c->prof_names.size()) return ELP_ERR_ARG;
  if (name) *name = c->prof_names[index].c_str();
  if (launches) *launches = c->prof_launches[index];
  if (total_ms) *total_ms = c->prof_ms[index];
  return 0;
}

}
```

elprep_amd/csrc/markdup.hip:

```cpp
#include "common.hpp"
#include "markdup_plan.hpp"

namespace elp {

constexpr uint32_t EMPTY = 0xFFFFFFFFu;
constexpr unsigned long long PB_EMPTY = ~0ull;

struct MdCols {
  uint64_t n;
  const int32_t *refid;
  const uint16_t *flag_in;
  const uint16_t *rgid;
  const uint16_t *rg_lib;
  const uint16_t *split;
  const int32_t *upos, *score;
  const uint64_t *qname_off;
  const uint8_t *qname;
};

__device__ __forceinline__ bool is_candidate(uint16_t f) { return (f & (F_UNMAPPED | F_SECONDARY | F_SUPPLEMENTARY)) == 0; }
__device__ __forceinline__ bool is_true_pair(uint16_t f) { return (f & (F_MULTIPLE | F_NEXT_UNMAPPED)) == F_MULTIPLE; }
__device__ __forceinline__ uint16_t lib_of(const MdCols &m, uint32_t i) {
  const uint16_t rg = m.rgid[i];
  return rg == ELP_NIL16 ? (uint16_t)ELP_NIL16 : m.rg_lib[rg];
}
__device__ __forceinline__ uint32_t ld_agent(const uint32_t *p) { return __hip_atomic_load(p, __ATOMIC_RELAXED, __HIP_MEMORY_SCOPE_AGENT); }
__device__ __forceinline__ unsigned long long ld_agent64(const unsigned long long *p) {
  return __hip_atomic_load(p, __ATOMIC_RELAXED, __HIP_MEMORY_SCOPE_AGENT);
}

__device__ __forceinline__ bool key_eq(const uint4 &a, const uint4 &b) { return a.x == b.x && a.y == b.y && a.z == b.z && a.w == b.w; }
__device__ __forceinline__ uint64_t frag_hash(const uint4 &k) {
  const uint64_t h = ((uint64_t)k.x << 32) | k.y;
  return mix64(mix64(h) ^ (((uint64_t)k.w << 32) | (uint64_t)k.z));
}

template <class Eq>
__device__ __forceinline__ uint32_t find_or_insert(uint32_t *table, uint64_t mask, uint64_t h, uint32_t i, Eq eq, uint64_t limit = ~0ull) {
  uint64_t s = h & mask;
  for (uint64_t probes = 0;; probes++) {
    if (probes > limit) return EMPTY;
    const uint32_t cur = atomicCAS(&table[s], EMPTY, i);
    if (cur == EMPTY) return i;
    if (cur == i || eq(cur, i)) return cur;
    s = (s + 1) & mask;
  }
}

__global__ __launch_bounds__(256) void k_frag_insert(MdCols m, const uint4 *__restrict__ fkey, const uint32_t *__restrict__ flist, uint32_t nf,
                                                     uint32_t *table, uint64_t mask, uint32_t *__restrict__ frep, unsigned long long *fbest) {
  const uint32_t j = blockIdx.x * blockDim.x + threadIdx.x;
  if (j >= nf) return;
  const uint32_t i = flist[j];
  const uint4 mine = fkey[i];
  const uint32_t rep = find_or_insert(table, mask, frag_hash(mine), i, [&](uint32_t a, uint32_t) { return key_eq(fkey[a], mine); });
  frep[i] = rep;
  atomicMax(&fbest[rep], (unsigned long long)(uint32_t)m.score[i]);
}
__global__ __launch_bounds__(256) void k_frag_bits(const uint32_t *__restrict__ table, uint64_t nwords, uint32_t *__restrict__ bits) {
  const uint64_t w = (uint64_t)blockIdx.x * blockDim.x + threadIdx.x;
  if (w >= nwords) return;
  const uint4 *t = reinterpret_cast<const uint4 *>(table + 32 * w);
  uint32_t b = 0;
#pragma unroll
  for (int k = 0; k < 8; k++) {
    const uint4 v = t[k];
    b |= (v.x != EMPTY ? 1u : 0u) << (4 * k) | (v.y != EMPTY ? 2u : 0u) << (4 * k) | (v.z != EMPTY ? 4u : 0u) << (4 * k) | (v.w != EMPTY ? 8u : 0u) << (4 * k);
  }
  bits[w] = b;
}
__device__ __forceinline__ void tournament(const MdCols &m, uint32_t *winner, uint32_t me) {
  uint32_t w = ld_agent(winner);
  for (;;) {
    if (w == EMPTY) {
      const uint32_t old = atomicCAS(winner, EMPTY, me);
      if (old == EMPTY) return;
      w = old;
      continue;
    }
    const int cq = qname_cmp(m.qname, m.qname_off, me, w);
    const bool better = cq < 0 || (cq == 0 && me > w);
    if (!better) return;
    const uint32_t old = atomicCAS(winner, w, me);
    if (old == w) return;
    w = old;
  }
}

__global__ __launch_bounds__(256) void k_frag_tie(MdCols m, const uint32_t *__restrict__ flist, uint32_t nf, const uint32_t *__restrict__ frep,
                                                  const unsigned long long *__restrict__ fbest, uint32_t *fwinner) {
  const uint32_t j = blockIdx.x * blockDim.x + threadIdx.x;
  if (j >= nf) return;
  const uint32_t i = flist[j];
  const uint32_t rep = frep[i];
  const unsigned long long b = fbest[rep];
  if ((b >> 63) || (unsigned long long)(uint32_t)m.score[i] != b) return;
  tournament(m, &fwinner[rep], (uint32_t)i);
}

__global__ __launch_bounds__(256) void k_frag_flag(MdCols m, const uint32_t *__restrict__ flist, uint32_t nf, const uint32_t *__restrict__ frep,
                                                   const unsigned long long *__restrict__ fbest, const uint32_t *__restrict__ fwinner,
                                                   uint16_t *__restrict__ flag_out) {
  const uint32_t j = blockIdx.x * blockDim.x + threadIdx.x;
  if (j >= nf) return;
  const uint32_t i = flist[j];
  const uint32_t rep = frep[i];
  const unsigned long long b = fbest[rep];
  const bool dup = (b >> 63) || (unsigned long long)(uint32_t)m.score[i] < b || fwinner[rep] != (uint32_t)i;
  if (dup) flag_out[i] = (uint16_t)(flag_out[i] | F_DUPLICATE);
}

struct PairKey { uint4 k1, k2; };
__device__ __forceinline__ PairKey pair_key(const uint4 &second, const uint4 &first) {
  const int32_t r1 = (int32_t)second.x, r2 = (int32_t)first.x, p1 = (int32_t)second.y, p2 = (int32_t)first.y;
  const bool v1 = second.z & 1u, v2 = first.z & 1u;
  const bool swap = r1 > r2 || (r1 == r2 && (p1 > p2 || (p1 == p2 && v1 && !v2)));
  return swap ? PairKey{first, second} : PairKey{second, first};
}
__device__ __forceinline__ bool pair_key_eq(const PairKey &a, const PairKey &b) {
  return a.k1.x == b.k1.x && a.k2.x == b.k2.x && a.k1.y == b.k1.y && a.k2.y == b.k2.y && a.k1.z == b.k1.z && ((a.k2.z ^ b.k2.z) & 1u) == 0 &&
         a.k1.w == b.k1.w;
}

__device__ __forceinline__ uint64_t pair_hash(const PairKey &k) {
  uint64_t h = mix64(((uint64_t)k.k1.x << 32) | k.k2.x);
  h = mix64(h ^ (((uint64_t)k.k1.y << 32) | k.k2.y));
  return mix64(h ^ (((uint64_t)k.k1.z << 1) | (k.k2.z & 1u)) ^ ((uint64_t)k.k1.w << 40));
}

__device__ __forceinline__ uint64_t qname_hash(const MdCols &m, uint32_t i) {
  const uint64_t o = m.qname_off[i];
  const uint32_t l = (uint32_t)(m.qname_off[i + 1] - o);
  uint64_t h = 0x9e3779b97f4a7c15ull ^ l;
  for (uint32_t k = 0; k < l; k += 8) h = (h ^ low_bytes(load8(m.qname + o + k), l - k)) * 0xff51afd7ed558ccdull + (h >> 29);
  return mix64(h ^ ((uint64_t)lib_of(m, i) << 48) ^ ((uint64_t)m.split[i] << 24));
}
__device__ __forceinline__ bool mate_key_eq(const MdCols &m, const uint4 *__restrict__ fkey, uint32_t a, const uint4 &kb, uint32_t b) {
  const uint4 ka = fkey[a];
  return (ka.z >> 1) == (kb.z >> 1) && ka.w == kb.w && qname_eq(m.qname, m.qname_off, a, b);
}
__device__ __forceinline__ bool is_mate_candidate(uint16_t f) { return is_candidate(f) && is_true_pair(f); }

enum : uint8_t { MC_NONE = 0, MC_TABLE = 1, MC_LEAD = 2, MC_FOLLOW = 3, MC_KIND = 3, MC_TABBED = 4  };
constexpr uint32_t MATE_BIG = 0xFFFFFFFEu;

__global__ __launch_bounds__(256) void k_bloom_coarse(const uint32_t *__restrict__ bloom, uint32_t n_lines, uint32_t *__restrict__ coarse) {
  const uint32_t line = blockIdx.x * 256 + threadIdx.x;
  bool nz = false;
  if (line < n_lines) {
    const uint4 *l = reinterpret_cast<const uint4 *>(bloom + (size_t)line * 16);
    const uint4 a = l[0], b = l[1], c2 = l[2], d = l[3];
    nz = (a.x | a.y | a.z | a.w | b.x | b.y | b.z | b.w | c2.x | c2.y | c2.z | c2.w | d.x | d.y | d.z | d.w) != 0;
  }
  const unsigned long long bits = __ballot(nz);
  if ((threadIdx.x & 63) == 0 && line < n_lines) {
    coarse[line >> 5] = (uint32_t)bits;
    coarse[(line >> 5) + 1] = (uint32_t)(bits >> 32);
  }
}

__device__ __forceinline__ void mate_table_insert(const MdCols &m, const uint4 *__restrict__ fkey, uint32_t i, uint64_t h, uint32_t *table, uint64_t mask, uint32_t *mate,
                                                  uint32_t *rep_of, uint32_t *err) {
  const uint4 mine = fkey[i];
  const uint32_t rep = find_or_insert(table, mask, h, i, [&](uint32_t a, uint32_t b) { return mate_key_eq(m, fkey, a, mine, b); }, mask);
  if (rep == EMPTY) atomicOr(&err[1], 2u);
  else if (rep != i) {
    rep_of[i] = rep;
    const uint32_t old = atomicCAS(&mate[rep], EMPTY, i);
    if (old == EMPTY) mate[i] = rep;
    else {
      rep_of[rep] = MATE_BIG;
      atomicOr(&err[1], 1u);
    }
  }
}
__global__ __launch_bounds__(256) void k_mate_table(MdCols m, const uint4 *__restrict__ fkey, const uint8_t *__restrict__ code, const uint32_t *__restrict__ hash32,
                                                    const uint32_t *__restrict__ hash_lo, const uint32_t *__restrict__ tab_list, const uint32_t *__restrict__ tab_cnt,
                                                    uint32_t cap, uint32_t *table, uint64_t mask, uint32_t *mate, uint32_t *rep_of, uint32_t *err) {
  __shared__ uint32_t first[65];
  if (threadIdx.x < 64) {
    const uint32_t c = tab_cnt[threadIdx.x * 16u];
    uint32_t incl = c;
    for (int d = 1; d < 64; d <<= 1) {
      const uint32_t up = __shfl_up(incl, d, 64);
      if ((int)threadIdx.x >= d) incl += up;
    }
    first[threadIdx.x + 1] = incl;
    if (threadIdx.x == 0) first[0] = 0;
  }
  __syncthreads();
  for (uint32_t g = blockIdx.x * 256u + threadIdx.x; g < first[64]; g += gridDim.x * 256u) {
    uint32_t lo = 0, hi = 64;
    while (hi - lo > 1) {
      const uint32_t mid = (lo + hi) >> 1;
      if (first[mid] <= g) lo = mid; else hi = mid;
    }
    const uint32_t i = tab_list[(size_t)lo * cap + (g - first[lo])];
    const uint64_t h = (code[i] & MC_KIND) == MC_TABLE ? ((uint64_t)hash32[i] << 32) | hash_lo[i] : qname_hash(m, i);
    mate_table_insert(m, fkey, i, h, table, mask, mate, rep_of, err);
  }
}

__global__ __launch_bounds__(256) void k_mate_pairs(MdCols m, const uint4 *__restrict__ fkey, uint8_t *__restrict__ code,
                                                    const uint32_t *__restrict__ hash32, const uint32_t *__restrict__ hash_lo, const uint32_t *__restrict__ bloom,
                                                    uint32_t bloom_mask, const uint32_t *__restrict__ coarse ,
                                                    uint32_t *table, uint64_t mask, uint32_t *mate, uint32_t *rep_of, uint32_t *err, int fixed,
                                                    uint64_t *__restrict__ pk, uint32_t *__restrict__ pv,
                                                    uint32_t *__restrict__ tab_list , uint32_t *tab_cnt, uint32_t tab_cap) {
  const uint64_t base = (uint64_t)blockIdx.x * (256 * MP_R) + threadIdx.x;
  uint8_t cd[MP_R];
  uint4 mine[MP_R], prev[MP_R];
  uint32_t hi[MP_R], hl[MP_R], bl[MP_R];
  int32_t sc[MP_R];
#pragma unroll
  for (int r = 0; r < MP_R; r++) {
    const uint64_t i = base + (uint64_t)r * 256;
    const bool in = i < m.n;
    cd[r] = in ? (uint8_t)(code[i] & MC_KIND) : (uint8_t)MC_NONE;
    mine[r] = in ? fkey[i] : make_uint4(0, 0, 0, 0);
    const uint32_t h0 = in ? hash32[i] : 0u, h1 = (in && i > 0) ? hash32[i - 1] : 0u;
    hi[r] = cd[r] == MC_LEAD ? h0 : h1;
    hl[r] = (in && cd[r] == MC_TABLE) ? hash_lo[i] : 0u;
  }
#pragma unroll
  for (int r = 0; r < MP_R; r++) {
    const uint64_t i = base + (uint64_t)r * 256;
    const bool cand = cd[r] != MC_NONE;
    bl[r] = ~0u;
    if (cand && cd[r] != MC_TABLE) {
      const uint32_t wi = (hi[r] >> 5) & bloom_mask, line = wi >> 4;
      bl[r] = (coarse && ((coarse[line >> 5] >> (line & 31u)) & 1u)) ? bloom[wi] : 0u;
    }
    const bool fol = cd[r] == MC_FOLLOW;
    prev[r] = fol ? fkey[i - 1] : make_uint4(0, 0, 0, 0);
    sc[r] = fol ? m.score[i] + m.score[i - 1] : 0;
  }
#pragma unroll
  for (int r = 0; r < MP_R; r++) {
    const uint64_t i = base + (uint64_t)r * 256;
    bool own = false, want_tab = false;
    uint64_t key = 0;
    if (cd[r] != MC_NONE) {
      const bool tab = cd[r] == MC_TABLE || ((bl[r] >> (hi[r] & 31u)) & 1u);
      if (!tab) {
        mate[i] = cd[r] == MC_LEAD ? (uint32_t)i + 1 : (uint32_t)i - 1;
        if (cd[r] == MC_FOLLOW) {
          if (fixed) {
            own = true;
            key = ((uint64_t)(uint32_t)sc[r] << 32) | (uint32_t)pair_hash(pair_key(mine[r], prev[r]));
          } else {
            code[i] = (uint8_t)(cd[r] | MC_TABBED);
          }
        }
      } else {
        code[i] = (uint8_t)(cd[r] | MC_TABBED);
        if (tab_list) want_tab = true;
        else mate_table_insert(m, fkey, (uint32_t)i, cd[r] == MC_TABLE ? ((uint64_t)hash32[i] << 32) | hl[r] : qname_hash(m, (uint32_t)i), table, mask, mate, rep_of, err);
      }
    }
    if (tab_list) {
      const unsigned long long tm = __ballot(want_tab);
      if (tm) {
        const int lane = threadIdx.x & 63, leader = __ffsll((long long)tm) - 1;
        const uint32_t li = blockIdx.x & 63u;
        uint32_t at = 0;
        if (lane == leader) at = atomicAdd(&tab_cnt[li * 16u], (uint32_t)__popcll(tm));
        at = __shfl(at, leader, 64) + (uint32_t)__popcll(tm & ((1ull << lane) - 1ull));
        if (want_tab) tab_list[(size_t)li * tab_cap + at] = (uint32_t)i;
      }
    }
    if (fixed) {
      const int next_owns = __shfl_down((int)own, 1, 64);
      if (own) {
        pk[i >> 1] = key;
        pv[i >> 1] = (uint32_t)i;
      } else if (!(threadIdx.x & 1u) && !next_owns && i < m.n) {
        pk[i >> 1] = 0xFFFFFFFF00000000ull | (uint32_t)mix64(i);
        pv[i >> 1] = EMPTY;
      }
    }
  }
}

__global__ __launch_bounds__(256) void k_big_collect(uint64_t n, const uint32_t *__restrict__ rep_of, uint32_t *mate, uint64_t *__restrict__ keys,
                                                     uint32_t *__restrict__ vals, uint32_t *count) {
  const uint64_t i = (uint64_t)blockIdx.x * 256 + threadIdx.x;
  if (i >= n) return;
  const uint32_t r = rep_of[i];
  if (r == EMPTY) return;
  uint32_t rep;
  if (r == MATE_BIG) rep = (uint32_t)i;
  else if (rep_of[r] == MATE_BIG) rep = r;
  else return;
  const uint32_t at = atomicAdd(count, 1u);
  keys[at] = ((uint64_t)rep << 32) | (uint64_t)i;
  vals[at] = (uint32_t)i;
  mate[i] = EMPTY;
}
__global__ __launch_bounds__(256) void k_big_pair(uint32_t cnt, const uint64_t *__restrict__ keys, uint32_t *mate) {
  const uint32_t j = blockIdx.x * 256 + threadIdx.x;
  if (j >= cnt) return;
  const uint32_t rep = (uint32_t)(keys[j] >> 32);
  if (j > 0 && (uint32_t)(keys[j - 1] >> 32) == rep) return;
  for (uint32_t k = j; k + 1 < cnt && (uint32_t)(keys[k + 1] >> 32) == rep; k += 2) {
    const uint32_t a = (uint32_t)keys[k], b = (uint32_t)keys[k + 1];
    mate[a] = b;
    mate[b] = a;
  }
}

__device__ __forceinline__ uint64_t pair_entry(const MdCols &m, const uint4 &later, const uint4 &earlier, uint32_t i, uint32_t mt) {
  return ((uint64_t)(uint32_t)(m.score[i] + m.score[mt]) << 32) | (uint32_t)pair_hash(pair_key(later, earlier));
}
__global__ __launch_bounds__(256) void k_pair_list_table(MdCols m, const uint4 *__restrict__ fkey, const uint32_t *__restrict__ mate,
                                                         const uint8_t *__restrict__ code, uint64_t *__restrict__ pk, uint32_t *__restrict__ pv,
                                                         uint32_t *np) {
  __shared__ uint64_t lk[PL_TILES * 256];
  __shared__ uint32_t lv[PL_TILES * 256];
  __shared__ uint32_t lcount, gbase;
  if (threadIdx.x == 0) lcount = 0;
  __syncthreads();
#pragma unroll 2
  for (int tile = 0; tile < PL_TILES; tile++) {
    const uint64_t i64 = ((uint64_t)blockIdx.x * PL_TILES + (uint64_t)tile) * 256 + threadIdx.x;
    const uint32_t i = (uint32_t)i64;
    const uint32_t mt = (i64 < m.n && (code[i64] & MC_TABBED)) ? mate[i] : EMPTY;
    const bool own = mt != EMPTY && mt < i;
    uint64_t key = 0;
    if (own) key = pair_entry(m, fkey[i], fkey[mt], i, mt);
    const unsigned long long mask = __ballot(own);
    if (mask) {
      const int lane = threadIdx.x & 63, leader = __ffsll((long long)mask) - 1;
      uint32_t at = 0;
      if (lane == leader) at = atomicAdd(&lcount, (uint32_t)__popcll(mask));
      at = __shfl(at, leader, 64);
      if (own) {
        at += (uint32_t)__popcll(mask & ((1ull << lane) - 1ull));
        lk[at] = key;
        lv[at] = i;
      }
    }
  }
  __syncthreads();
  if (threadIdx.x == 0) gbase = lcount ? atomicAdd(np, lcount) : 0u;
  __syncthreads();
  for (uint32_t k = threadIdx.x; k < lcount; k += 256) {
    pk[gbase + k] = lk[k];
    pv[gbase + k] = lv[k];
  }
}

__global__ __launch_bounds__(256) void k_pair_list_lists(MdCols m, const uint4 *__restrict__ fkey, const uint32_t *__restrict__ mate, const uint32_t *__restrict__ tab_list,
                                                         const uint32_t *__restrict__ tab_cnt, uint32_t cap, uint64_t *__restrict__ pk, uint32_t *__restrict__ pv, uint32_t *np) {
  __shared__ uint32_t first[65];
  if (threadIdx.x < 64) {
    uint32_t incl = tab_cnt[threadIdx.x * 16u];
    for (int d = 1; d < 64; d <<= 1) {
      const uint32_t up = __shfl_up(incl, d, 64);
      if ((int)threadIdx.x >= d) incl += up;
    }
    first[threadIdx.x + 1] = incl;
    if (threadIdx.x == 0) first[0] = 0;
  }
  __syncthreads();
  __shared__ uint64_t lk[PL_TILES * 256];
  __shared__ uint32_t lv[PL_TILES * 256];
  __shared__ uint32_t lcount, gbase;
  const uint32_t total = first[64], chunk = PL_TILES * 256u;
  for (uint32_t c0 = blockIdx.x * chunk; c0 < total; c0 += gridDim.x * chunk) {
    if (threadIdx.x == 0) lcount = 0;
    __syncthreads();
#pragma unroll 2
    for (int tile = 0; tile < PL_TILES; tile++) {
      const uint32_t g = c0 + (uint32_t)tile * 256u + threadIdx.x;
      uint32_t i = 0, mt = EMPTY;
      if (g < total) {
        uint32_t lo = 0, hi = 64;
        while (hi - lo > 1) {
          const uint32_t mid = (lo + hi) >> 1;
          if (first[mid] <= g) lo = mid; else hi = mid;
        }
        i = tab_list[(size_t)lo * cap + (g - first[lo])];
        mt = mate[i];
      }
      const bool own = mt != EMPTY && mt < i;
      uint64_t key = 0;
      if (own) key = pair_entry(m, fkey[i], fkey[mt], i, mt);
      const unsigned long long mask = __ballot(own);
      if (mask) {
        const int lane = threadIdx.x & 63, leader = __ffsll((long long)mask) - 1;
        uint32_t at = 0;
        if (lane == leader) at = atomicAdd(&lcount, (uint32_t)__popcll(mask));
        at = __shfl(at, leader, 64);
        if (own) {
          at += (uint32_t)__popcll(mask & ((1ull << lane) - 1ull));
          lk[at] = key;
          lv[at] = i;
        }
      }
    }
    __syncthreads();
    if (threadIdx.x == 0) gbase = lcount ? atomicAdd(np, lcount) : 0u;
    __syncthreads();
    for (uint32_t k = threadIdx.x; k < lcount; k += 256) {
      pk[gbase + k] = lk[k];
      pv[gbase + k] = lv[k];
    }
    __syncthreads();
  }
}

__device__ __forceinline__ uint32_t pair_bucket(uint64_t key, int sbits, int bbits) {
  return bbits ? ((uint32_t)key & ((1u << sbits) - 1u)) >> (sbits - bbits) : 0u;
}
__global__ __launch_bounds__(256) void k_pair_bounds(const uint64_t *__restrict__ ks, const uint32_t *__restrict__ np, int sbits, int bbits,
                                                     uint32_t *__restrict__ bstart, uint32_t *__restrict__ bend) {
  const uint32_t n = *np;
  const uint32_t j = blockIdx.x * 256 + threadIdx.x;
  if (j >= n) return;
  const uint32_t b = pair_bucket(ks[j], sbits, bbits);
  if (j == 0 || pair_bucket(ks[j - 1], sbits, bbits) != b) bstart[b] = j;
  if (j + 1 == n || pair_bucket(ks[j + 1], sbits, bbits) != b) bend[b] = j + 1;
}

__device__ __forceinline__ PairKey pair_key_of(const uint4 *__restrict__ fkey, const uint32_t *__restrict__ mate, uint32_t owner) {
  return pair_key(fkey[owner], fkey[mate[owner]]);
}
__device__ __forceinline__ void tournament_lds(const MdCols &m, uint32_t *winner, uint32_t me) {
  uint32_t w = *(volatile uint32_t *)winner;
  for (;;) {
    if (w != EMPTY) {
      const int cq = qname_cmp(m.qname, m.qname_off, me, w);
      if (!(cq < 0 || (cq == 0 && me > w))) return;
    }
    const uint32_t old = atomicCAS(winner, w, me);
    if (old == w) return;
    w = old;
  }
}
__device__ __forceinline__ void pair_lost(const MdCols &m, const uint32_t *__restrict__ mate, uint32_t o, uint32_t w, uint32_t *__restrict__ pair_win,
                                          uint16_t *__restrict__ flag_out) {
  const uint32_t mt = mate[o];
  pair_win[o] = w;
  flag_out[o] = (uint16_t)(flag_out[o] | F_DUPLICATE);
  flag_out[mt] = (uint16_t)(flag_out[mt] | F_DUPLICATE);
}

constexpr int PB_ECAP = 1024;

__device__ __forceinline__ int pb_slot(const MdCols &m, const uint4 *__restrict__ fkey, const uint32_t *__restrict__ mate,
                                       unsigned long long *s_key, uint32_t tmask, uint32_t h32, uint32_t o, bool insert) {
  uint32_t idx = (h32 * 0x9E3779B1u) >> 16 & tmask;
  const unsigned long long mine = ((unsigned long long)h32 << 32) | o;
  for (uint32_t probes = 0; probes <= tmask; probes++, idx = (idx + 1) & tmask) {
    unsigned long long cur = insert ? atomicCAS(&s_key[idx], PB_EMPTY, mine) : s_key[idx];
    if (cur == PB_EMPTY) { if (insert) return (int)idx; else continue; }
    if (cur == mine) return (int)idx;
    if ((uint32_t)(cur >> 32) == h32 && pair_key_eq(pair_key_of(fkey, mate, (uint32_t)cur), pair_key_of(fkey, mate, o))) return (int)idx;
  }
  return -1;
}

__global__ __launch_bounds__(PB_THREADS) void k_pair_bucket(MdCols m, const uint4 *__restrict__ fkey, const uint32_t *__restrict__ mate,
                                                     const uint64_t *__restrict__ ks, uint32_t *__restrict__ vs,
                                                     const uint32_t *__restrict__ bstart, const uint32_t *__restrict__ bend, int cap_slots,
                                                     uint32_t *__restrict__ pair_win, uint16_t *__restrict__ flag_out, int inv_end ) {
  __shared__ unsigned long long s_key[PB_CAP];
  __shared__ uint32_t s_best[PB_CAP], s_win[PB_CAP];
  __shared__ uint16_t s_slot[PB_ECAP];
  __shared__ uint32_t s_full, s_min, s_h;
  const uint32_t start = bstart[blockIdx.x], end = inv_end ? ~bend[blockIdx.x] : bend[blockIdx.x];
  if (end <= start) return;
  const uint32_t cnt = end - start;
  const uint32_t t = threadIdx.x;
  if (cnt == 1) return;
  uint32_t T = 2;
  while (T < 2 * cnt && T < (uint32_t)cap_slots) T <<= 1;
  const uint32_t tmask = T - 1;
  for (uint32_t k = t; k < T; k += PB_THREADS) { s_key[k] = PB_EMPTY; s_best[k] = 0; s_win[k] = EMPTY; }
  if (t == 0) s_full = 0;
  __syncthreads();
  ks += start;
  vs += start;
  for (uint32_t e = t; e < cnt; e += PB_THREADS) {
    const uint64_t key = ks[e];
    const uint32_t o = vs[e];
    if (o == EMPTY) continue;
    const int slot = pb_slot(m, fkey, mate, s_key, tmask, (uint32_t)key, o, true);
    if (slot < 0) { s_full = 1; break; }
    atomicMax(&s_best[slot], (uint32_t)(key >> 32));
    if (e < PB_ECAP) s_slot[e] = (uint16_t)slot;
  }
  __syncthreads();
  if (!s_full) {
    for (uint32_t e = t; e < cnt; e += PB_THREADS) {
      const uint64_t key = ks[e];
      const uint32_t o = vs[e];
      if (o == EMPTY) continue;
      const int slot = e < PB_ECAP ? (int)s_slot[e] : pb_slot(m, fkey, mate, s_key, tmask, (uint32_t)key, o, false);
      if ((uint32_t)(key >> 32) == s_best[slot]) tournament_lds(m, &s_win[slot], o);
    }
    __syncthreads();
    for (uint32_t e = t; e < cnt; e += PB_THREADS) {
      const uint32_t o = vs[e];
      if (o == EMPTY) continue;
      const int slot = e < PB_ECAP ? (int)s_slot[e] : pb_slot(m, fkey, mate, s_key, tmask, (uint32_t)ks[e], o, false);
      const uint32_t w = s_win[slot];
      if (w != o) pair_lost(m, mate, o, w, pair_win, flag_out);
    }
    return;
  }
  for (;;) {
    __syncthreads();
    if (t == 0) { s_min = EMPTY; s_best[0] = 0; s_win[0] = EMPTY; }
    __syncthreads();
    for (uint32_t e = t; e < cnt; e += PB_THREADS) {
      const uint32_t o = vs[e];
      if (o != EMPTY) atomicMin(&s_min, o);
    }
    __syncthreads();
    const uint32_t rep = s_min;
    if (rep == EMPTY) return;
    for (uint32_t e = t; e < cnt; e += PB_THREADS)
      if (vs[e] == rep) s_h = (uint32_t)ks[e];
    __syncthreads();
    const uint32_t rh = s_h;
    const PairKey rk = pair_key_of(fkey, mate, rep);
    for (uint32_t e = t; e < cnt; e += PB_THREADS) {
      const uint32_t o = vs[e];
      if (o != EMPTY && (uint32_t)ks[e] == rh && pair_key_eq(rk, pair_key_of(fkey, mate, o))) atomicMax(&s_best[0], (uint32_t)(ks[e] >> 32));
    }
    __syncthreads();
    for (uint32_t e = t; e < cnt; e += PB_THREADS) {
      const uint32_t o = vs[e];
      if (o != EMPTY && (uint32_t)ks[e] == rh && (uint32_t)(ks[e] >> 32) == s_best[0] && pair_key_eq(rk, pair_key_of(fkey, mate, o)))
        tournament_lds(m, &s_win[0], o);
    }
    __syncthreads();
    for (uint32_t e = t; e < cnt; e += PB_THREADS) {
      const uint32_t o = vs[e];
      if (o != EMPTY && (uint32_t)ks[e] == rh && pair_key_eq(rk, pair_key_of(fkey, mate, o))) {
        if (s_win[0] != o) pair_lost(m, mate, o, s_win[0], pair_win, flag_out);
        vs[e] = EMPTY;
      }
    }
  }
}

__device__ __forceinline__ uint32_t next_lane(uint32_t x) { return (uint32_t)__builtin_amdgcn_update_dpp(0, (int)x, 0x130 , 0xf, 0xf, false); }
__device__ __forceinline__ uint64_t next_lane64(uint64_t x) { return (uint64_t)next_lane((uint32_t)x) | ((uint64_t)next_lane((uint32_t)(x >> 32)) << 32); }

struct FrontCols {
  uint64_t n;
  const int32_t *refid, *pos;
  const uint16_t *flag;
  const uint8_t *state;
  const uint16_t *rgid, *rg_lib, *split;
  const uint64_t *cigar_off;
  const uint32_t *cigar;
  const uint64_t *qname_off;
  const uint8_t *qname;
  uint32_t n_ref;
  int pos_bits;
};
__device__ __forceinline__ int32_t unclipped_pos(uint16_t f, int32_t p, uint64_t c0, uint64_t c1, const uint32_t *__restrict__ cigar, uint32_t o0, uint32_t o1,
                                                 uint32_t o2, uint32_t o3) {
  if ((f & (F_UNMAPPED | F_SECONDARY | F_SUPPLEMENTARY)) != 0) return 0;
  int32_t up = p;
  const uint64_t nop = c1 - c0;
  auto at = [&](uint64_t k) __attribute__((always_inline)) -> uint32_t { return k == 0 ? o0 : (k == 1 ? o1 : (k == 2 ? o2 : (k == 3 ? o3 : cigar[c0 + k]))); };
  if (nop) {
    if (f & F_REVERSED) {
      int32_t clipped = 1;
      up--;
      for (uint64_t k = nop; k-- > 0;) {
        const uint32_t c = at(k), op = c & 0xF;
        const int32_t isclip = (op == OP_S || op == OP_H) ? 1 : 0;
        const int32_t isref = op_consumes_ref(op) ? 1 : 0;
        clipped *= isclip;
        up += (isref | clipped) * (int32_t)(c >> 4);
      }
    } else {
      for (uint64_t k = 0; k < nop; k++) {
        const uint32_t c = at(k), op = c & 0xF;
        if (!(op == OP_S || op == OP_H)) break;
        up -= (int32_t)(c >> 4);
      }
    }
  }
  return up;
}
__device__ __forceinline__ uint16_t flag_in_of(uint16_t f, uint8_t state) { return state == 2 ? (uint16_t)(f | F_SECONDARY) : f; }

constexpr int FLI_CAP = 4096;
__global__ __launch_bounds__(256) void k_frag_list(FrontCols m, uint4 *__restrict__ fkey, uint32_t *__restrict__ flist, uint32_t *nf,
                                                   unsigned long long *__restrict__ fbest, uint32_t *__restrict__ fwinner) {
  __shared__ uint32_t lq[FLI_CAP];
  __shared__ uint32_t lcount, gbase;
  if (threadIdx.x == 0) lcount = 0;
  __syncthreads();
  const uint64_t nchunks = (m.n + FLI_CHUNK - 1) / FLI_CHUNK;
  for (uint64_t ch = blockIdx.x; ch < nchunks; ch += gridDim.x) {
    const uint64_t i0 = (ch * 256 + threadIdx.x) * 8;
    uint4 fv = make_uint4(0, 0, 0, 0);
    uint2 sv = make_uint2(0, 0);
    if (i0 < m.n) {
      fv = *reinterpret_cast<const uint4 *>(m.flag + i0);
      sv = *reinterpret_cast<const uint2 *>(m.state + i0);
    }
    const uint32_t fw[4] = {fv.x, fv.y, fv.z, fv.w};
    const uint64_t st8 = (uint64_t)sv.x | ((uint64_t)sv.y << 32);
    uint32_t fm = 0;
#pragma unroll
    for (int k = 0; k < 8; k++) {
      const uint16_t f = flag_in_of((uint16_t)(fw[k >> 1] >> (16 * (k & 1))), (uint8_t)(st8 >> (8 * k)));
      if (i0 + (uint64_t)k < m.n && is_candidate(f) && !is_true_pair(f)) fm |= 1u << k;
    }
    if (fm) {
      uint32_t at = atomicAdd(&lcount, (uint32_t)__popc(fm));
      for (; fm; fm &= fm - 1u) lq[at++] = (uint32_t)i0 + (uint32_t)(__ffs((int)fm) - 1);
    }
    __syncthreads();
    const uint32_t cnt = lcount;
    if (cnt + FLI_CHUNK <= (uint32_t)FLI_CAP && ch + gridDim.x < nchunks) continue;
    if (threadIdx.x == 0) gbase = cnt ? atomicAdd(nf, cnt) : 0u;
    __syncthreads();
    for (uint32_t k = threadIdx.x; k < cnt; k += 256) {
      const uint32_t i = lq[k];
      const uint16_t f = m.flag[i], rg = m.rgid[i];
      const uint64_t c0 = m.cigar_off[i], c1 = m.cigar_off[i + 1];
      const uint64_t nop = c1 - c0;
      const uint32_t o0 = nop > 0 ? m.cigar[c0] : 0u, o1 = nop > 1 ? m.cigar[c0 + 1] : 0u, o2 = nop > 2 ? m.cigar[c0 + 2] : 0u, o3 = nop > 3 ? m.cigar[c0 + 3] : 0u;
      const uint16_t lib = rg == ELP_NIL16 ? (uint16_t)ELP_NIL16 : m.rg_lib[rg];
      const int32_t up = unclipped_pos(f, m.pos[i], c0, c1, m.cigar, o0, o1, o2, o3);
      fkey[i] = make_uint4((uint32_t)m.refid[i], (uint32_t)up, ((uint32_t)lib << 1) | ((f & F_REVERSED) ? 1u : 0u), (uint32_t)m.split[i]);
      fbest[i] = 0;
      fwinner[i] = EMPTY;
      flist[gbase + k] = i;
    }
    __syncthreads();
    if (threadIdx.x == 0) lcount = 0;
    __syncthreads();
  }
}

template <bool ADAPT>
__global__ __launch_bounds__(MF_THREADS) void k_md_front(FrontCols m, const int32_t *__restrict__ score, int32_t *__restrict__ upos_out, uint64_t *__restrict__ key_out,
                                                         uint4 *fkey, uint8_t *__restrict__ code, uint32_t *__restrict__ hash32, uint32_t *__restrict__ hash_lo, uint32_t *bloom,
                                                         uint32_t bloom_mask, uint32_t *n_table, const uint32_t *__restrict__ ftable, const uint32_t *__restrict__ fbits,
                                                         uint64_t fmask , unsigned long long *fbest, uint32_t *__restrict__ mate,
                                                         uint32_t *__restrict__ pair_win, uint64_t *__restrict__ pk, uint32_t *__restrict__ pv, uint32_t *np,
                                                         uint32_t nfixed, int optimistic) {
  const uint64_t base = (uint64_t)blockIdx.x * MF_RECS;
  const uint32_t t = threadIdx.x, lane = t & 63u, u = 63u * (t >> 6) + lane;
  const int64_t a_s = (int64_t)base - 2 + (int64_t)u;
  const bool own_rec = a_s >= 0 && (uint64_t)a_s < m.n;
  const bool valid = a_s >= 0 && (uint64_t)a_s + 1 < m.n;
  const uint64_t a = own_rec ? (uint64_t)a_s : 0;
  const uint16_t fa_st = m.flag[a], ra = m.rgid[a], sa = m.split[a];
  const uint8_t sta = m.state[a];
  const int32_t r = m.refid[a], p = m.pos[a], sc = score[a];
  const uint64_t oa = m.qname_off[a], oa1 = m.qname_off[a + 1];
  const uint64_t c0 = m.cigar_off[a], c1 = m.cigar_off[a + 1];
  const uint32_t la = (uint32_t)(oa1 - oa);
  const uint64_t nop = c1 - c0;
  const uint16_t lia = ra == ELP_NIL16 ? (uint16_t)ELP_NIL16 : m.rg_lib[ra];
  const uint8_t *pa = m.qname + oa;
  const uint64_t a0 = load8(pa), a1 = load8(pa + 8), a2 = load8(pa + 16), a3 = load8(pa + 24);
  const uint32_t o0 = nop > 0 ? m.cigar[c0] : 0u, o1 = nop > 1 ? m.cigar[c0 + 1] : 0u, o2 = nop > 2 ? m.cigar[c0 + 2] : 0u, o3 = nop > 3 ? m.cigar[c0 + 3] : 0u;
  const uint16_t fa = flag_in_of(fa_st, sta);
  const int32_t up = unclipped_pos(fa_st, p, c0, c1, m.cigar, o0, o1, o2, o3);
  const uint4 mine = make_uint4((uint32_t)r, (uint32_t)up, ((uint32_t)lia << 1) | ((fa & F_REVERSED) ? 1u : 0u), (uint32_t)sa);
  const uint64_t w0 = la > 0 ? low_bytes(a0, la) : 0ull, w1 = la > 8 ? low_bytes(a1, la - 8) : 0ull, w2 = la > 16 ? low_bytes(a2, la - 16) : 0ull,
                 w3 = la > 24 ? low_bytes(a3, la - 24) : 0ull;
  const uint32_t mcand = own_rec && is_mate_candidate(fa) ? 1u : 0u;
  const uint32_t nA = next_lane(mcand | ((uint32_t)lia << 1)), nL = next_lane(la);
  const uint32_t nS = next_lane((uint32_t)sa);
  const uint64_t b0 = next_lane64(w0), b1 = next_lane64(w1), b2 = next_lane64(w2), b3 = next_lane64(w3);
  const uint64_t n_oa = next_lane64(oa);
  bool join = valid && lane < 63u && mcand && (nA & 1u) && (uint16_t)(nA >> 1) == lia && (uint16_t)nS == sa && nL == la;
  if (join) {
    join = ((w0 ^ b0) | (w1 ^ b1) | (w2 ^ b2) | (w3 ^ b3)) == 0;
    const uint8_t *pb = m.qname + n_oa;
    for (uint32_t k = 32; join && k < la; k += 8) join = low_bytes(load8(pa + k), la - k) == low_bytes(load8(pb + k), la - k);
  }
  __shared__ uint8_t s_join[320];
  __shared__ uint4 s_fk[316];
  __shared__ int32_t s_sc[316];
  if (lane < 63u) {
    s_join[u] = join;
    s_fk[u] = mine;
    s_sc[u] = sc;
  }
  __syncthreads();
  const bool mine_rec = own_rec && lane < 63u && u >= 2u && u < 2u + (uint32_t)MF_RECS;
  const uint64_t i = a;
  uint8_t cd = MC_NONE;
  if (mine_rec) {
    if (ADAPT) {
      const uint64_t ru = sta ? (uint64_t)m.n_ref + 1 : (r < 0 ? (uint64_t)m.n_ref : (uint64_t)(uint32_t)r);
      key_out[i] = (ru << (m.pos_bits + 1)) | ((uint64_t)(uint32_t)p << 1) | ((fa_st & F_REVERSED) ? 1ull : 0ull);
      upos_out[i] = up;
    }
    if (!(is_candidate(fa) && !is_true_pair(fa))) fkey[i] = mine;
    pair_win[i] = EMPTY;
  }
  const uint8_t *j = s_join + u;
  if (mine_rec && mcand) {
    const bool nx = j[0], pv_ = j[-1];
    cd = MC_TABLE;
    if (nx && !pv_ && !j[1]) cd = MC_LEAD;
    else if (pv_ && !nx && !j[-2]) cd = MC_FOLLOW;
    if (cd != MC_FOLLOW) {
      uint64_t h = 0x9e3779b97f4a7c15ull ^ la;
      const uint64_t K = 0xff51afd7ed558ccdull;
      if (la > 0) h = (h ^ w0) * K + (h >> 29);
      if (la > 8) h = (h ^ w1) * K + (h >> 29);
      if (la > 16) h = (h ^ w2) * K + (h >> 29);
      if (la > 24) h = (h ^ w3) * K + (h >> 29);
      for (uint32_t k = 32; k < la; k += 8) h = (h ^ low_bytes(load8(pa + k), la - k)) * K + (h >> 29);
      h = mix64(h ^ ((uint64_t)lia << 48) ^ ((uint64_t)sa << 24));
      const uint32_t hi = (uint32_t)(h >> 32);
      hash32[i] = hi;
      if (cd == MC_TABLE) hash_lo[i] = (uint32_t)h;
      if (cd != MC_LEAD) atomicOr(&bloom[(hi >> 5) & bloom_mask], 1u << (hi & 31u));
    }
  }
  if (mine_rec) code[i] = cd;
  const unsigned long long tb = __ballot(cd == MC_TABLE);
  if (lane == 0 && tb) atomicAdd(&n_table[((blockIdx.x * 5u + (t >> 6)) & 63u) * 16u], (uint32_t)__popcll(tb));
  if (cd != MC_NONE && fmask) {
    uint64_t s = frag_hash(mine) & fmask;
    for (;; s = (s + 1) & fmask) {
      if (!((fbits[s >> 5] >> (s & 31)) & 1u)) break;
      const uint32_t c2 = ftable[s];
      if (key_eq(fkey[c2], mine)) {
        atomicMax(&fbest[c2], 1ull << 63);
        break;
      }
    }
  }
  if (mine_rec) mate[i] = !optimistic ? EMPTY : (cd == MC_LEAD ? (uint32_t)i + 1 : (cd == MC_FOLLOW ? (uint32_t)i - 1 : EMPTY));
  if (optimistic && mine_rec) {
    if (cd == MC_FOLLOW) {
      pk[i >> 1] = ((uint64_t)(uint32_t)(sc + s_sc[u - 1]) << 32) | (uint32_t)pair_hash(pair_key(mine, s_fk[u - 1]));
      pv[i >> 1] = (uint32_t)i;
    } else if (!(i & 1ull) && !(j[0] && !j[1] && !j[-1])) {
      pk[i >> 1] = 0xFFFFFFFF00000000ull | (uint32_t)mix64(i);
      pv[i >> 1] = EMPTY;
    }
    if (i == 0) *np = nfixed;
  }
}

struct MdBufs {
  MdCols m;
  uint32_t *table, *rep, *flist, *winner, *bloom, *coarse, *hash32, *tab_list, *hash_lo;
  unsigned long long *best;
  uint4 *fkey;
  uint8_t *code;
  uint64_t *pk;
  uint32_t *pv, *ftable, *fbits;
  uint32_t *nf_dev, *np_dev, *n_table_dev;
  uint32_t *rep_of;
};
constexpr size_t MD_CTRS = 16 + 64 * 16;

static int md_carve(elp_ctx *c, const MdScratch &L, MdBufs *b) {
  b->m = MdCols{c->n, c->refid.p, c->flag.p, c->rgid.p, c->rg_lib.p, c->split.p, c->upos.p, c->score.p, c->qname_off.p, c->qname.p};
  ELP_TRY(scratch(c, 0, L.table, &b->table));
  ELP_TRY(scratch(c, 2, L.best, &b->best));
  ELP_TRY(scratch(c, 3, L.winner, &b->winner));
  ELP_TRY(scratch(c, 5, L.fkey, &b->fkey));
  ELP_TRY(ensure(c, c->md_ctr, MD_CTRS));
  ELP_TRY(scratch(c, 1, L.words1, &b->rep));
  b->flist = b->rep + L.flist;
  b->nf_dev = c->md_ctr.p, b->np_dev = c->md_ctr.p + 1, b->n_table_dev = c->md_ctr.p + 16;
  b->rep_of = c->pair_win.p;
  return 0;
}

static int md_frag_list(elp_ctx *c, const MdSizes &S, const MdBufs &B, const FrontCols &fc) {
  hipStream_t st = c->stream;
  ELP_HIP(c, hipMemsetAsync(c->md_ctr.p, 0, MD_CTRS * sizeof(uint32_t), st));
  ELP_TRY(mailbox(c));
  ELP_LAUNCH(c, "md_frag_list", k_frag_list, dim3(S.frag_list_grid(c->n_cu)), dim3(256), 0, fc, B.fkey, B.flist, B.nf_dev, B.best, B.winner);
  ELP_HIP(c, hipMemcpyAsync(c->mail, B.nf_dev, 4, hipMemcpyDeviceToHost, st));
  ELP_HIP(c, hipEventRecord(c->mail_ev, st));
  return 0;
}

static int md_front(elp_ctx *c, const MdSizes &S, const MdScratch &L, MdBufs &B, const FrontCols &fc, bool fuse_adapt, uint32_t *nf_out) {
  hipStream_t st = c->stream;
  ELP_TRY(scratch(c, 6, L.words6, &B.bloom));
  B.coarse = B.bloom + L.coarse, B.hash32 = B.bloom + L.hash32, B.tab_list = B.bloom + L.tab_list, B.hash_lo = B.bloom + L.hash_lo;
  B.code = reinterpret_cast<uint8_t *>(B.bloom + L.code);
  ELP_HIP(c, hipMemsetAsync(B.bloom, 0, S.bw * sizeof(uint32_t), st));
  ELP_HIP(c, elp::event_wait(c->mail_ev));
  const uint32_t nf = *nf_out = c->mail[0];
  const uint64_t Tf = frag_table_size(nf, S.T);
  const MdScratch::Pairs P = L.pairs(Tf);
  ELP_TRY(scratch(c, 7, P.words64, &B.pk));
  uint32_t *const w7 = reinterpret_cast<uint32_t *>(B.pk);
  B.pv = w7 + P.pv, B.ftable = w7 + P.ftable, B.fbits = w7 + P.fbits;
  if (nf) {
    ELP_HIP(c, hipMemsetAsync(B.ftable, 0xFF, Tf * sizeof(uint32_t), st));
    ELP_LAUNCH(c, "md_frag_insert", k_frag_insert, dim3(blocks_for(nf, 256)), dim3(256), 0, B.m, (const uint4 *)B.fkey, (const uint32_t *)B.flist, nf, B.ftable, Tf - 1, B.rep, B.best);
    ELP_LAUNCH(c, "md_frag_bits", k_frag_bits, dim3(blocks_for(Tf / 32, 256)), dim3(256), 0, (const uint32_t *)B.ftable, Tf / 32, B.fbits);
  }
  const auto front = fuse_adapt ? k_md_front<true> : k_md_front<false>;
  ELP_LAUNCH(c, "md_front", front, dim3(S.front_grid), dim3(MF_THREADS), 0, fc, (const int32_t *)c->score.p, c->upos.p, c->key.p, B.fkey, B.code, B.hash32, B.hash_lo, B.bloom,
             (uint32_t)(S.bw - 1), B.n_table_dev, (const uint32_t *)B.ftable, (const uint32_t *)B.fbits, nf ? Tf - 1 : (uint64_t)0, B.best, c->mate.p, c->pair_win.p, B.pk, B.pv, B.np_dev, S.nfx,
             c->tune.mate_path == 0 ? 1 : 0);
  return 0;
}

static int md_fragments(elp_ctx *c, const MdBufs &B, uint32_t nf, uint32_t *n_tab_out) {
  hipStream_t st = c->stream;
  if (nf) {
    const unsigned fgrid = blocks_for(nf, 256);
    ELP_LAUNCH(c, "md_frag_tie", k_frag_tie, dim3(fgrid), dim3(256), 0, B.m, (const uint32_t *)B.flist, nf, (const uint32_t *)B.rep, (const unsigned long long *)B.best, B.winner);
    ELP_LAUNCH(c, "md_frag_flag", k_frag_flag, dim3(fgrid), dim3(256), 0, B.m, (const uint32_t *)B.flist, nf, (const uint32_t *)B.rep, (const unsigned long long *)B.best,
               (const uint32_t *)B.winner, c->flag.p);
  }
  uint32_t n_tab64[64 * 16], adapt_word[ADAPT_WORDS] = {0, 0, 0, 0, 0, 0};
  ELP_HIP(c, hipMemcpyAsync(n_tab64, B.n_table_dev, sizeof n_tab64, hipMemcpyDeviceToHost, st));
  const bool adapt_read = c->derived.adapt_pending;
  if (adapt_read) ELP_HIP(c, hipMemcpyAsync(adapt_word, c->adapt_err.p, sizeof adapt_word, hipMemcpyDeviceToHost, st));
  ELP_HIP(c, elp::stream_wait(st));
  if (adapt_read) adapt_note(c, adapt_word);
  if (c->derived.adapt_bad_qual) return adapt_quality_error(c);
  *n_tab_out = 0;
  for (int k = 0; k < 64; k++) *n_tab_out += n_tab64[k * 16];
  return 0;
}

static int md_mates(elp_ctx *c, const MdSizes &S, const MdBufs &B, const MatePlan &P, uint32_t n_tab, bool *big) {
  hipStream_t st = c->stream;
  const uint64_t n = S.n;
  ELP_HIP(c, hipMemsetAsync(c->mate.p, 0xFF, n * sizeof(uint32_t), st));
  if (n_tab) ELP_LAUNCH(c, "md_bloom_coarse", k_bloom_coarse, dim3(S.coarse_grid), dim3(256), 0, (const uint32_t *)B.bloom, (uint32_t)(S.bw / 16), B.coarse);
  uint32_t e[4] = {0, 0, 0, 0};
  for (uint64_t Tm = P.Tm;; Tm = S.T) {
    ELP_HIP(c, hipMemsetAsync(B.table, 0xFF, Tm * sizeof(uint32_t), st));
    ELP_HIP(c, hipMemsetD32Async(reinterpret_cast<hipDeviceptr_t>(B.np_dev), (int)(uint32_t)P.nfixed, 1, st));
    if (P.listed) ELP_HIP(c, hipMemsetAsync(B.n_table_dev, 0, 64 * 16 * sizeof(uint32_t), st));
    ELP_LAUNCH(c, "md_mate_pairs", k_mate_pairs, dim3(S.mate_grid), dim3(256), 0, B.m, (const uint4 *)B.fkey, B.code, (const uint32_t *)B.hash32, (const uint32_t *)B.hash_lo,
               (const uint32_t *)B.bloom, (uint32_t)(S.bw - 1), (const uint32_t *)(n_tab ? B.coarse : nullptr), B.table, Tm - 1, c->mate.p, B.rep_of, c->err_flag.p, P.fixed ? 1 : 0, B.pk,
               B.pv, P.listed ? B.tab_list : (uint32_t *)nullptr, B.n_table_dev, S.tab_cap);
    if (P.listed)
      ELP_LAUNCH(c, "md_mate_table", k_mate_table, dim3(blocks_for(P.list_n, 256)), dim3(256), 0, B.m, (const uint4 *)B.fkey, (const uint8_t *)B.code, (const uint32_t *)B.hash32,
                 (const uint32_t *)B.hash_lo, (const uint32_t *)B.tab_list, (const uint32_t *)B.n_table_dev, S.tab_cap, B.table, Tm - 1, c->mate.p, B.rep_of, c->err_flag.p);
    ELP_TRY(fetch_err(c, e));
    if (!(e[1] & 2u)) break;
    if (Tm == S.T) return set_error(c, ELP_ERR_HIP, "mark duplicates: mate table overflow");
    ELP_HIP(c, hipMemsetAsync(c->err_flag.p + 1, 0, 4, st));
    ELP_HIP(c, hipMemsetAsync(c->mate.p, 0xFF, n * sizeof(uint32_t), st));
    ELP_HIP(c, hipMemsetAsync(B.rep_of, 0xFF, n * sizeof(uint32_t), st));
  }
  *big = e[1] != 0;
  return 0;
}

static int md_big_groups(elp_ctx *c, const MdSizes &S, const MdScratch &L, const MdBufs &B) {
  hipStream_t st = c->stream;
  ELP_HIP(c, hipMemsetAsync(c->err_flag.p + 1, 0, 4, st));
  uint64_t *bk, *ks;
  uint32_t *bv, *vs, *cnt_dev = c->err_flag.p + 3;
  ELP_TRY(scratch(c, 2, L.big, &bk));
  ELP_TRY(scratch(c, 3, L.big, &bv));
  ELP_HIP(c, hipMemsetAsync(cnt_dev, 0, 4, st));
  ELP_LAUNCH(c, "md_big_collect", k_big_collect, dim3(S.grid), dim3(256), 0, S.n, (const uint32_t *)B.rep_of, c->mate.p, bk, bv, cnt_dev);
  uint32_t cnt = 0;
  ELP_HIP(c, hipMemcpyAsync(&cnt, cnt_dev, 4, hipMemcpyDeviceToHost, st));
  ELP_HIP(c, elp::stream_wait(st));
  ELP_HIP(c, hipMemsetAsync(cnt_dev, 0, 4, st));
  ProfScope ps(c, "md_big_");
  ELP_TRY(radix_sort_pairs(c, bk, bv, bk + S.n, bv + S.n, cnt, &ks, &vs));
  ELP_LAUNCH(c, "md_big_pair", k_big_pair, dim3(blocks_for(cnt, 256)), dim3(256), 0, cnt, (const uint64_t *)ks, c->mate.p);
  return 0;
}

static int md_pairs(elp_ctx *c, const MdSizes &S, const MdScratch &L, const MdBufs &B, const MatePlan &P) {
  hipStream_t st = c->stream;
  uint32_t *bounds;
  ELP_TRY(scratch(c, 1, L.bounds_words, &bounds));
  const bool folded = S.ndig > 0;
  ELP_HIP(c, hipMemsetAsync(bounds, folded ? 0xFF : 0, 2 * S.nb * sizeof(uint32_t), st));
  if (!P.fast) {
    ELP_HIP(c, hipMemsetAsync(c->pair_win.p, 0xFF, S.n * sizeof(uint32_t), st));
    if (P.listed)
      ELP_LAUNCH(c, "md_pair_list", k_pair_list_lists, dim3(blocks_for(P.list_n, 256 * PL_TILES)), dim3(256), 0, B.m, (const uint4 *)B.fkey, (const uint32_t *)c->mate.p, (const uint32_t *)B.tab_list,
                 (const uint32_t *)B.n_table_dev, S.tab_cap, B.pk, B.pv, B.np_dev);
    else
      ELP_LAUNCH(c, "md_pair_list", k_pair_list_table, dim3(S.list_grid), dim3(256), 0, B.m, (const uint4 *)B.fkey, (const uint32_t *)c->mate.p, (const uint8_t *)B.code, B.pk, B.pv,
                 B.np_dev);
  }
  uint64_t *ks = B.pk;
  uint32_t *vs = B.pv;
  if (folded) {
    ProfScope ps(c, "md_pair_");
    ELP_TRY(radix_sort_pairs_low(c, B.pk, B.pv, B.pk + S.npmax, B.pv + S.npmax, S.npmax, S.ndig, &ks, &vs, nullptr, false, B.np_dev,
                                 RadixBounds{bounds, bounds + S.nb, (uint32_t)((1ull << S.sbits) - 1ull), S.sbits - S.bbits}));
  } else {
    ELP_LAUNCH(c, "md_pair_bounds", k_pair_bounds, dim3(S.bounds_grid), dim3(256), 0, (const uint64_t *)ks, (const uint32_t *)B.np_dev, S.sbits, S.bbits, bounds, bounds + S.nb);
  }
  ELP_LAUNCH(c, "md_pair_bucket", k_pair_bucket, dim3((unsigned)S.nb), dim3(PB_THREADS), 0, B.m, (const uint4 *)B.fkey, (const uint32_t *)c->mate.p, (const uint64_t *)ks, vs,
             (const uint32_t *)bounds, (const uint32_t *)(bounds + S.nb), std::min(c->tune.pair_table_slots, PB_CAP), c->pair_win.p, c->flag.p, folded ? 1 : 0);
  return 0;
}

static int markdup_impl(elp_ctx *c) {
  const uint64_t n = c->n;
  ELP_TRY(ensure(c, c->mate, n + 1));
  ELP_TRY(ensure(c, c->pair_win, n + 1));
  if (n == 0) { ELP_TRY(ensure_adapted(c, true)); c->derived.marked = true; return 0; }
  const bool fuse_adapt = !c->derived.adapted();
  int pos_bits = 1;
  if (fuse_adapt) ELP_TRY(adapt_begin(c, &pos_bits));
  else ELP_TRY(ensure_adapted(c, false));
  const MdSizes S(n);
  const MdScratch L(S);
  MdBufs B;
  ELP_TRY(md_carve(c, L, &B));
  const FrontCols fc{n, c->refid.p, c->pos.p, c->flag.p, c->has_sr.p, c->rgid.p, c->rg_lib.p, c->split.p, c->cigar_off.p, c->cigar.p, c->qname_off.p, c->qname.p,
                     (uint32_t)c->n_ref, pos_bits};
  ELP_TRY(md_frag_list(c, S, B, fc));
  if (fuse_adapt) ELP_TRY(adapt_scores(c));
  uint32_t nf = 0, n_tab = 0;
  ELP_TRY(md_front(c, S, L, B, fc, fuse_adapt, &nf));
  if (fuse_adapt) c->derived.keys = c->derived.scores = true;
  ELP_TRY(sort_presort(c));
  ELP_TRY(md_fragments(c, B, nf, &n_tab));
  const MatePlan P = mate_plan(n, n_tab, c->tune.mate_path, S.T);
  bool big = false;
  if (!P.fast) ELP_TRY(md_mates(c, S, B, P, n_tab, &big));
  if (big) ELP_TRY(md_big_groups(c, S, L, B));
  ELP_TRY(md_pairs(c, S, L, B, P));
  c->radix_check_pending = true;
  c->derived.marked = true;
  return 0;
}

}

extern "C" int elp_mark_duplicates(elp_ctx *c, int also_opticals) {
  (void)also_opticals;
  if (!c) return ELP_ERR_ARG;
  ELP_HIP(c, hipSetDevice(c->device));
  c->derived.drop_marked();
  return elp::markdup_impl(c);
}
```

elprep_amd/csrc/markdup_plan.hpp:

```cpp
#pragma once
#include <algorithm>
#include <cstddef>
#include <cstdint>

namespace elp {

constexpr int MP_R = 1;
constexpr int PL_TILES = 8;
constexpr int PB_THREADS = 256;
constexpr int PB_TARGET = 384;
constexpr int PB_CAP = 1024;
constexpr int FLI_CHUNK = 2048;
constexpr int MF_THREADS = 320, MF_RECS = 312;

inline unsigned md_blocks(uint64_t n, unsigned per_block) { return (unsigned)((n + per_block - 1) / per_block); }

inline uint64_t table_size_for(uint64_t n) {
  uint64_t t = 1024;
  while (t < 2 * n + 16) t <<= 1;
  return t;
}

struct MdSizes {
  uint64_t n, T;
  int bbits, ndig, sbits;
  size_t nb;
  uint64_t bw;
  uint32_t tab_cap;
  uint64_t npmax;
  uint32_t nfx;
  unsigned grid, frag_list_blocks, front_grid, mate_grid, coarse_grid, list_grid, bounds_grid;
  explicit MdSizes(uint64_t records) : n(records), T(table_size_for(records)), bbits(0), bw(1024), npmax(records + 2), nfx((uint32_t)((records + 1) / 2)) {
    while (bbits < 24 && ((n / 2 + 1) >> bbits) > (uint64_t)PB_TARGET) bbits++;
    ndig = (bbits + 7) / 8;
    sbits = 8 * ndig;
    nb = (size_t)1 << bbits;
    while (bw < n / 16 && bw < (1u << 20)) bw <<= 1;
    grid = md_blocks(n, 256);
    frag_list_blocks = md_blocks(n, FLI_CHUNK);
    front_grid = md_blocks(n, MF_RECS);
    mate_grid = md_blocks(n, 256 * MP_R);
    coarse_grid = md_blocks(bw / 16, 256);
    list_grid = md_blocks(n, 256 * PL_TILES);
    bounds_grid = md_blocks(npmax, 256);
    tab_cap = (uint32_t)((mate_grid + 63) / 64) * 256u * MP_R;
  }
  unsigned frag_list_grid(int n_cu) const { return std::min<unsigned>(frag_list_blocks, (unsigned)n_cu * 8); }
};

struct MdScratch {
  size_t table, best, winner, fkey, big;
  size_t flist, words1, bounds_words;
  size_t coarse, hash32, code, tab_list, hash_lo, words6;
  uint64_t npmax;
  explicit MdScratch(const MdSizes &s) : npmax(s.npmax) {
    const size_t n = (size_t)s.n;
    table = (size_t)s.T;
    best = winner = n + 16;
    fkey = n + 8;
    big = 2 * n + 8;
    flist = n + 8;
    words1 = flist + n + 8;
    bounds_words = 2 * s.nb + 8;
    coarse = (size_t)s.bw;
    hash32 = coarse + (size_t)s.bw / 512 + 16;
    code = hash32 + n + 8;
    tab_list = code + 8 + (n + 16) / 4;
    hash_lo = tab_list + 64 * (size_t)s.tab_cap + 8;
    words6 = hash_lo + 8 + n + 16;
  }
  struct Pairs { size_t pv, ftable, fbits, words64; };
  Pairs pairs(uint64_t Tf) const {
    const size_t pv = 4 * (size_t)npmax, ftable = pv + 2 * (size_t)npmax, fbits = ftable + (size_t)Tf;
    return Pairs{pv, ftable, fbits, (fbits + (size_t)Tf / 32 + 64) / 2 + 8};
  }
};

inline uint64_t frag_table_size(uint32_t nf, uint64_t T) { return nf ? std::min<uint64_t>(T, table_size_for(4ull * nf)) : 0; }

struct MatePlan {
  bool fixed, fast, listed;
  uint64_t nfixed, Tm, list_n;
};
inline MatePlan mate_plan(uint64_t n, uint32_t n_tab, int mate_path, uint64_t T) {
  const bool fixed = (uint64_t)n_tab < n / 8 && mate_path == 0;
  return MatePlan{fixed, fixed && n_tab == 0, fixed && n_tab != 0, fixed ? (n + 1) / 2 : 0,
                  fixed ? std::min<uint64_t>(T, table_size_for(std::min<uint64_t>(n, 4ull * n_tab + 1024))) : T, std::min<uint64_t>(n, 2ull * n_tab + 4096)};
}

}
```

Measured before the change: 2495.

## Run quality score kernel on a side stream beside markdup front pass

```diff
diff --git a/elprep_amd/csrc/adapt.hip b/elprep_amd/csrc/adapt.hip
--- a/elprep_amd/csrc/adapt.hip
+++ b/elprep_amd/csrc/adapt.hip
@@ -250,10 +250,10 @@
   return ((L / 4u) % 4u) != 0;
 }
 template <int R>
-static int score_uniform_launch(elp_ctx *c) {
+static int score_uniform_launch(elp_ctx *c, unsigned per_cu) {
   const uint32_t L = c->uniform_len;
   const size_t dyn = (size_t)SU_WAVES * ((size_t)64 * L + 16);
-  const unsigned per_cu = (unsigned)std::max<size_t>(1, (160 * 1024) / (dyn + 256));
+  if (!per_cu) per_cu = (unsigned)std::max<size_t>(1, (160 * 1024) / (dyn + 256));
   const uint64_t ngroups = (c->n + 63) / 64;
   const unsigned grid = (unsigned)std::min<uint64_t>((ngroups + SU_WAVES - 1) / SU_WAVES, (uint64_t)c->n_cu * per_cu);
   ELP_HIP(c, hipFuncSetAttribute(reinterpret_cast<const void *>(&k_score_uniform<R>), hipFuncAttributeMaxDynamicSharedMemorySize, (int)dyn));
@@ -271,9 +271,9 @@
   c->apply_recs_lmax = (int)L;
   return 0;
 }
-static int score_uniform(elp_ctx *c) {
+static int score_uniform(elp_ctx *c, unsigned per_cu) {
   switch ((c->uniform_len + 15u) / 16u) {
-#define ELP_SU(R) case R: return score_uniform_launch<R>(c);
+#define ELP_SU(R) case R: return score_uniform_launch<R>(c, per_cu);
     ELP_SU(1) ELP_SU(2) ELP_SU(3) ELP_SU(4) ELP_SU(5) ELP_SU(6) ELP_SU(7) ELP_SU(8) ELP_SU(9) ELP_SU(10) ELP_SU(11) ELP_SU(12) ELP_SU(13) ELP_SU(14)
     ELP_SU(15) ELP_SU(16)
 #undef ELP_SU
@@ -404,7 +404,7 @@
   *pos_bits_out = kw.pos_bits;
   return 0;
 }
-int adapt_scores(elp_ctx *c) {
+int adapt_scores(elp_ctx *c, bool beside) {
   const uint64_t n = c->n;
   if (!n) return 0;
   if (!c->qual_bytes) {
@@ -414,7 +414,7 @@
   }
   ELP_TRY(ensure_uniform_len(c));
   if (c->uniform_len && score_uniform_ok(c->uniform_len) && c->tune.score_kernel != 1) {
-    ELP_TRY(score_uniform(c));
+    ELP_TRY(score_uniform(c, beside ? 1u : 0u));
   } else {
     ELP_HIP(c, hipMemsetAsync(c->score.p, 0, n * sizeof(int32_t), c->stream));
     const unsigned grid = (unsigned)std::min<uint64_t>(flat_steps<ScoreBody>(c->qual_bytes), (uint64_t)c->n_cu * 4);
@@ -423,6 +423,19 @@
   }
   c->derived.adapt_pending = true;
   return 0;
+}
+int adapt_scores_beside(elp_ctx *c, bool *pending) {
+  *pending = false;
+  ELP_TRY(score_lane_fork(c));
+  int rc;
+  {
+    StreamScope on_lane(c, c->score_stream);
+    rc = adapt_scores(c, true);
+  }
+  *pending = c->derived.adapt_pending;
+  c->derived.adapt_pending = false;
+  const int rd = score_lane_done(c);
+  return rc != 0 ? rc : rd;
 }
 int ensure_adapted(elp_ctx *c, bool check_quals) {
   if (c->derived.adapted()) {
diff --git a/elprep_amd/csrc/common.hpp b/elprep_amd/csrc/common.hpp
--- a/elprep_amd/csrc/common.hpp
+++ b/elprep_amd/csrc/common.hpp
@@ -201,6 +201,9 @@
   uint64_t *presort_ks = nullptr;
   int presort_idx_bits = 0;
 
+  hipStream_t score_stream = nullptr;
+  hipEvent_t score_ev = nullptr, score_done = nullptr;
+
   elp::DVec<uint16_t> snap_flag;
   elp::DVec<uint8_t> snap_qual;
   uint64_t snap_n = 0, snap_qual_bytes = 0;
@@ -216,6 +219,7 @@
     int bgzf_weak_guess = 0;
     int score_kernel = 0;
     int mate_path = 0;
+    int score_lane = 1;
     int radix_tile = 0;
     int sort_pairs = 0;
     int tie_rounds = 0;
@@ -279,7 +283,16 @@
   ~ProfScope() { c->prof_prefix = saved; }
 };
 
-#define ELP_HIP(ctx, call)                                                                             \
+struct StreamScope {
+  elp_ctx *c;
+  hipStream_t saved;
+  StreamScope(elp_ctx *ctx, hipStream_t st) : c(ctx), saved(ctx->stream) { ctx->stream = st; }
+  StreamScope(const StreamScope &) = delete;
+  StreamScope &operator=(const StreamScope &) = delete;
+  ~StreamScope() { c->stream = saved; }
+};
+
+#define ELP_HIP(ctx, call)                                                                           \
   do {                                                                                                 \
     hipError_t e__ = (call);                                                                           \
     if (e__ != hipSuccess)                                                                             \
@@ -443,7 +456,11 @@
 int ensure_adapted(elp_ctx *c, bool check_quals = true);
 int ensure_keys(elp_ctx *c);
 int adapt_begin(elp_ctx *c, int *pos_bits);
-int adapt_scores(elp_ctx *c);
+int adapt_scores(elp_ctx *c, bool beside = false);
+int adapt_scores_beside(elp_ctx *c, bool *pending);
+int score_lane_fork(elp_ctx *c);
+int score_lane_done(elp_ctx *c);
+int score_lane_join(elp_ctx *c);
 int mailbox(elp_ctx *c);
 int side_lane(elp_ctx *c, int lane, elp_ctx **out);
 int side_join(elp_ctx *c, int lane);
diff --git a/elprep_amd/csrc/ctx.hip b/elprep_amd/csrc/ctx.hip
--- a/elprep_amd/csrc/ctx.hip
+++ b/elprep_amd/csrc/ctx.hip
@@ -193,6 +193,22 @@
 int side_join(elp_ctx *c, int lane) {
   ELP_HIP(c, hipEventRecord(c->side_done[lane], c->side[lane]->stream));
   ELP_HIP(c, hipStreamWaitEvent(c->stream, c->side_done[lane], 0));
+  return 0;
+}
+int score_lane_fork(elp_ctx *c) {
+  if (!c->score_stream) ELP_HIP(c, hipStreamCreateWithFlags(&c->score_stream, hipStreamNonBlocking));
+  if (!c->score_ev) ELP_HIP(c, hipEventCreateWithFlags(&c->score_ev, hipEventDisableTiming));
+  if (!c->score_done) ELP_HIP(c, hipEventCreateWithFlags(&c->score_done, hipEventDisableTiming));
+  ELP_HIP(c, hipEventRecord(c->score_ev, c->stream));
+  ELP_HIP(c, hipStreamWaitEvent(c->score_stream, c->score_ev, 0));
+  return 0;
+}
+int score_lane_done(elp_ctx *c) {
+  ELP_HIP(c, hipEventRecord(c->score_done, c->score_stream));
+  return 0;
+}
+int score_lane_join(elp_ctx *c) {
+  ELP_HIP(c, hipStreamWaitEvent(c->stream, c->score_done, 0));
   return 0;
 }
 void prof_merge_side(elp_ctx *c) {
@@ -311,6 +327,12 @@
     if (c->side_ev[lane]) (void)hipEventDestroy(c->side_ev[lane]);
     if (c->side_done[lane]) (void)hipEventDestroy(c->side_done[lane]);
   }
+  if (c->score_stream) {
+    (void)elp::stream_wait(c->score_stream);
+    (void)hipStreamDestroy(c->score_stream);
+  }
+  if (c->score_ev) (void)hipEventDestroy(c->score_ev);
+  if (c->score_done) (void)hipEventDestroy(c->score_done);
   if (c->mail) (void)hipHostFree(c->mail);
   if (c->mail_ev) (void)hipEventDestroy(c->mail_ev);
   for (int k = 0; k < 2; k++) {
@@ -606,6 +628,9 @@
   } else if (k == "mate_path") {
     if (value != 0 && value != 2) return set_error(c, ELP_ERR_ARG, "elp_set_tuning: mate_path is 0 (the library decides) or 2 (every candidate through the table)");
     c->tune.mate_path = v;
+  } else if (k == "score_lane") {
+    if (value != 0 && value != 1) return set_error(c, ELP_ERR_ARG, "elp_set_tuning: score_lane is 1 (the score kernel beside the front pass) or 0 (in line)");
+    c->tune.score_lane = v;
   } else if (k == "tie_rounds") c->tune.tie_rounds = v;
   else if (k == "radix_tile") c->tune.radix_tile = v;
   else if (k == "sort_pairs") c->tune.sort_pairs = v;
diff --git a/elprep_amd/csrc/markdup.hip b/elprep_amd/csrc/markdup.hip
--- a/elprep_amd/csrc/markdup.hip
+++ b/elprep_amd/csrc/markdup.hip
@@ -47,15 +47,21 @@
   }
 }
 
-__global__ __launch_bounds__(256) void k_frag_insert(MdCols m, const uint4 *__restrict__ fkey, const uint32_t *__restrict__ flist, uint32_t nf,
-                                                     uint32_t *table, uint64_t mask, uint32_t *__restrict__ frep, unsigned long long *fbest) {
+__global__ __launch_bounds__(256) void k_frag_insert(const uint4 *__restrict__ fkey, const uint32_t *__restrict__ flist, uint32_t nf, uint32_t *table, uint64_t mask,
+                                                     uint32_t *__restrict__ frep) {
   const uint32_t j = blockIdx.x * blockDim.x + threadIdx.x;
   if (j >= nf) return;
   const uint32_t i = flist[j];
   const uint4 mine = fkey[i];
   const uint32_t rep = find_or_insert(table, mask, frag_hash(mine), i, [&](uint32_t a, uint32_t) { return key_eq(fkey[a], mine); });
   frep[i] = rep;
-  atomicMax(&fbest[rep], (unsigned long long)(uint32_t)m.score[i]);
+}
+__global__ __launch_bounds__(256) void k_frag_best(const int32_t *__restrict__ score, const uint32_t *__restrict__ flist, uint32_t nf, const uint32_t *__restrict__ frep,
+                                                   unsigned long long *fbest) {
+  const uint32_t j = blockIdx.x * blockDim.x + threadIdx.x;
+  if (j >= nf) return;
+  const uint32_t i = flist[j];
+  atomicMax(&fbest[frep[i]], (unsigned long long)(uint32_t)score[i]);
 }
 __global__ __launch_bounds__(256) void k_frag_bits(const uint32_t *__restrict__ table, uint64_t nwords, uint32_t *__restrict__ bits) {
   const uint64_t w = (uint64_t)blockIdx.x * blockDim.x + threadIdx.x;
@@ -211,7 +217,6 @@
   uint8_t cd[MP_R];
   uint4 mine[MP_R], prev[MP_R];
   uint32_t hi[MP_R], hl[MP_R], bl[MP_R];
-  int32_t sc[MP_R];
 #pragma unroll
   for (int r = 0; r < MP_R; r++) {
     const uint64_t i = base + (uint64_t)r * 256;
@@ -233,7 +238,6 @@
     }
     const bool fol = cd[r] == MC_FOLLOW;
     prev[r] = fol ? fkey[i - 1] : make_uint4(0, 0, 0, 0);
-    sc[r] = fol ? m.score[i] + m.score[i - 1] : 0;
   }
 #pragma unroll
   for (int r = 0; r < MP_R; r++) {
@@ -247,7 +251,7 @@
         if (cd[r] == MC_FOLLOW) {
           if (fixed) {
             own = true;
-            key = ((uint64_t)(uint32_t)sc[r] << 32) | (uint32_t)pair_hash(pair_key(mine[r], prev[r]));
+            key = pair_entry_word((uint32_t)pair_hash(pair_key(mine[r], prev[r])));
           } else {
             code[i] = (uint8_t)(cd[r] | MC_TABBED);
           }
@@ -275,7 +279,7 @@
         pk[i >> 1] = key;
         pv[i >> 1] = (uint32_t)i;
       } else if (!(threadIdx.x & 1u) && !next_owns && i < m.n) {
-        pk[i >> 1] = 0xFFFFFFFF00000000ull | (uint32_t)mix64(i);
+        pk[i >> 1] = pair_hole_word((uint32_t)mix64(i));
         pv[i >> 1] = EMPTY;
       }
     }
@@ -309,9 +313,7 @@
   }
 }
 
-__device__ __forceinline__ uint64_t pair_entry(const MdCols &m, const uint4 &later, const uint4 &earlier, uint32_t i, uint32_t mt) {
-  return ((uint64_t)(uint32_t)(m.score[i] + m.score[mt]) << 32) | (uint32_t)pair_hash(pair_key(later, earlier));
-}
+__device__ __forceinline__ uint64_t pair_entry(const uint4 &later, const uint4 &earlier) { return pair_entry_word((uint32_t)pair_hash(pair_key(later, earlier))); }
 __global__ __launch_bounds__(256) void k_pair_list_table(MdCols m, const uint4 *__restrict__ fkey, const uint32_t *__restrict__ mate,
                                                          const uint8_t *__restrict__ code, uint64_t *__restrict__ pk, uint32_t *__restrict__ pv,
                                                          uint32_t *np) {
@@ -327,7 +329,7 @@
     const uint32_t mt = (i64 < m.n && (code[i64] & MC_TABBED)) ? mate[i] : EMPTY;
     const bool own = mt != EMPTY && mt < i;
     uint64_t key = 0;
-    if (own) key = pair_entry(m, fkey[i], fkey[mt], i, mt);
+    if (own) key = pair_entry(fkey[i], fkey[mt]);
     const unsigned long long mask = __ballot(own);
     if (mask) {
       const int lane = threadIdx.x & 63, leader = __ffsll((long long)mask) - 1;
@@ -385,7 +387,7 @@
       }
       const bool own = mt != EMPTY && mt < i;
       uint64_t key = 0;
-      if (own) key = pair_entry(m, fkey[i], fkey[mt], i, mt);
+      if (own) key = pair_entry(fkey[i], fkey[mt]);
       const unsigned long long mask = __ballot(own);
       if (mask) {
         const int lane = threadIdx.x & 63, leader = __ffsll((long long)mask) - 1;
@@ -446,17 +448,21 @@
   flag_out[mt] = (uint16_t)(flag_out[mt] | F_DUPLICATE);
 }
 
-constexpr int PB_ECAP = 1024;
+__device__ __forceinline__ uint32_t pair_sum(const MdCols &m, const uint32_t *__restrict__ mate, uint32_t o) { return (uint32_t)(m.score[o] + m.score[mate[o]]); }
 
 __device__ __forceinline__ int pb_slot(const MdCols &m, const uint4 *__restrict__ fkey, const uint32_t *__restrict__ mate,
-                                       unsigned long long *s_key, uint32_t tmask, uint32_t h32, uint32_t o, bool insert) {
+                                       unsigned long long *s_key, uint32_t tmask, uint32_t h32, uint32_t o, bool insert, uint32_t *first = nullptr) {
   uint32_t idx = (h32 * 0x9E3779B1u) >> 16 & tmask;
   const unsigned long long mine = ((unsigned long long)h32 << 32) | o;
+  if (first) *first = o;
   for (uint32_t probes = 0; probes <= tmask; probes++, idx = (idx + 1) & tmask) {
     unsigned long long cur = insert ? atomicCAS(&s_key[idx], PB_EMPTY, mine) : s_key[idx];
     if (cur == PB_EMPTY) { if (insert) return (int)idx; else continue; }
     if (cur == mine) return (int)idx;
-    if ((uint32_t)(cur >> 32) == h32 && pair_key_eq(pair_key_of(fkey, mate, (uint32_t)cur), pair_key_of(fkey, mate, o))) return (int)idx;
+    if ((uint32_t)(cur >> 32) == h32 && pair_key_eq(pair_key_of(fkey, mate, (uint32_t)cur), pair_key_of(fkey, mate, o))) {
+      if (first) *first = (uint32_t)cur;
+      return (int)idx;
+    }
   }
   return -1;
 }
@@ -469,6 +475,7 @@
   __shared__ uint32_t s_best[PB_CAP], s_win[PB_CAP];
   __shared__ uint16_t s_slot[PB_ECAP];
   __shared__ uint32_t s_full, s_min, s_h;
+  static_assert(sizeof s_key + sizeof s_best + sizeof s_win + sizeof s_slot + 12 <= pair_bucket_lds(), "markdup_plan.hpp: pair_bucket_lds");
   const uint32_t start = bstart[blockIdx.x], end = inv_end ? ~bend[blockIdx.x] : bend[blockIdx.x];
   if (end <= start) return;
   const uint32_t cnt = end - start;
@@ -477,7 +484,7 @@
   uint32_t T = 2;
   while (T < 2 * cnt && T < (uint32_t)cap_slots) T <<= 1;
   const uint32_t tmask = T - 1;
-  for (uint32_t k = t; k < T; k += PB_THREADS) { s_key[k] = PB_EMPTY; s_best[k] = 0; s_win[k] = EMPTY; }
+  for (uint32_t k = t; k < T; k += PB_THREADS) { s_key[k] = PB_EMPTY; s_best[k] = 0; s_win[k] = PB_SINGLE; }
   if (t == 0) s_full = 0;
   __syncthreads();
   ks += start;
@@ -486,27 +493,31 @@
     const uint64_t key = ks[e];
     const uint32_t o = vs[e];
     if (o == EMPTY) continue;
-    const int slot = pb_slot(m, fkey, mate, s_key, tmask, (uint32_t)key, o, true);
+    uint32_t first;
+    const int slot = pb_slot(m, fkey, mate, s_key, tmask, pair_word_hash(key), o, true, &first);
     if (slot < 0) { s_full = 1; break; }
-    atomicMax(&s_best[slot], (uint32_t)(key >> 32));
     if (e < PB_ECAP) s_slot[e] = (uint16_t)slot;
+    if (first == o) continue;
+    const uint32_t sum = pair_sum(m, mate, o), sum_first = pair_sum(m, mate, first);
+    atomicMax(&s_best[slot], max(sum, sum_first));
+    s_win[slot] = EMPTY;
   }
   __syncthreads();
   if (!s_full) {
     for (uint32_t e = t; e < cnt; e += PB_THREADS) {
-      const uint64_t key = ks[e];
       const uint32_t o = vs[e];
       if (o == EMPTY) continue;
-      const int slot = e < PB_ECAP ? (int)s_slot[e] : pb_slot(m, fkey, mate, s_key, tmask, (uint32_t)key, o, false);
-      if ((uint32_t)(key >> 32) == s_best[slot]) tournament_lds(m, &s_win[slot], o);
+      const int slot = e < PB_ECAP ? (int)s_slot[e] : pb_slot(m, fkey, mate, s_key, tmask, pair_word_hash(ks[e]), o, false);
+      if (*(volatile uint32_t *)&s_win[slot] == PB_SINGLE) continue;
+      if (pair_sum(m, mate, o) == s_best[slot]) tournament_lds(m, &s_win[slot], o);
     }
     __syncthreads();
     for (uint32_t e = t; e < cnt; e += PB_THREADS) {
       const uint32_t o = vs[e];
       if (o == EMPTY) continue;
-      const int slot = e < PB_ECAP ? (int)s_slot[e] : pb_slot(m, fkey, mate, s_key, tmask, (uint32_t)ks[e], o, false);
+      const int slot = e < PB_ECAP ? (int)s_slot[e] : pb_slot(m, fkey, mate, s_key, tmask, pair_word_hash(ks[e]), o, false);
       const uint32_t w = s_win[slot];
-      if (w != o) pair_lost(m, mate, o, w, pair_win, flag_out);
+      if (w != PB_SINGLE && w != o) pair_lost(m, mate, o, w, pair_win, flag_out);
     }
     return;
   }
@@ -528,12 +539,12 @@
     const PairKey rk = pair_key_of(fkey, mate, rep);
     for (uint32_t e = t; e < cnt; e += PB_THREADS) {
       const uint32_t o = vs[e];
-      if (o != EMPTY && (uint32_t)ks[e] == rh && pair_key_eq(rk, pair_key_of(fkey, mate, o))) atomicMax(&s_best[0], (uint32_t)(ks[e] >> 32));
+      if (o != EMPTY && pair_word_hash(ks[e]) == rh && pair_key_eq(rk, pair_key_of(fkey, mate, o))) atomicMax(&s_best[0], pair_sum(m, mate, o));
     }
     __syncthreads();
     for (uint32_t e = t; e < cnt; e += PB_THREADS) {
       const uint32_t o = vs[e];
-      if (o != EMPTY && (uint32_t)ks[e] == rh && (uint32_t)(ks[e] >> 32) == s_best[0] && pair_key_eq(rk, pair_key_of(fkey, mate, o)))
+      if (o != EMPTY && pair_word_hash(ks[e]) == rh && pair_key_eq(rk, pair_key_of(fkey, mate, o)) && pair_sum(m, mate, o) == s_best[0])
         tournament_lds(m, &s_win[0], o);
     }
     __syncthreads();
@@ -645,7 +656,7 @@
 }
 
 template <bool ADAPT>
-__global__ __launch_bounds__(MF_THREADS) void k_md_front(FrontCols m, const int32_t *__restrict__ score, int32_t *__restrict__ upos_out, uint64_t *__restrict__ key_out,
+__global__ __launch_bounds__(MF_THREADS) void k_md_front(FrontCols m, int32_t *__restrict__ upos_out, uint64_t *__restrict__ key_out,
                                                          uint4 *fkey, uint8_t *__restrict__ code, uint32_t *__restrict__ hash32, uint32_t *__restrict__ hash_lo, uint32_t *bloom,
                                                          uint32_t bloom_mask, uint32_t *n_table, const uint32_t *__restrict__ ftable, const uint32_t *__restrict__ fbits,
                                                          uint64_t fmask , unsigned long long *fbest, uint32_t *__restrict__ mate,
@@ -659,7 +670,7 @@
   const uint64_t a = own_rec ? (uint64_t)a_s : 0;
   const uint16_t fa_st = m.flag[a], ra = m.rgid[a], sa = m.split[a];
   const uint8_t sta = m.state[a];
-  const int32_t r = m.refid[a], p = m.pos[a], sc = score[a];
+  const int32_t r = m.refid[a], p = m.pos[a];
   const uint64_t oa = m.qname_off[a], oa1 = m.qname_off[a + 1];
   const uint64_t c0 = m.cigar_off[a], c1 = m.cigar_off[a + 1];
   const uint32_t la = (uint32_t)(oa1 - oa);
@@ -686,11 +697,9 @@
   }
   __shared__ uint8_t s_join[320];
   __shared__ uint4 s_fk[316];
-  __shared__ int32_t s_sc[316];
   if (lane < 63u) {
     s_join[u] = join;
     s_fk[u] = mine;
-    s_sc[u] = sc;
   }
   __syncthreads();
   const bool mine_rec = own_rec && lane < 63u && u >= 2u && u < 2u + (uint32_t)MF_RECS;
@@ -743,10 +752,10 @@
   if (mine_rec) mate[i] = !optimistic ? EMPTY : (cd == MC_LEAD ? (uint32_t)i + 1 : (cd == MC_FOLLOW ? (uint32_t)i - 1 : EMPTY));
   if (optimistic && mine_rec) {
     if (cd == MC_FOLLOW) {
-      pk[i >> 1] = ((uint64_t)(uint32_t)(sc + s_sc[u - 1]) << 32) | (uint32_t)pair_hash(pair_key(mine, s_fk[u - 1]));
+      pk[i >> 1] = pair_entry_word((uint32_t)pair_hash(pair_key(mine, s_fk[u - 1])));
       pv[i >> 1] = (uint32_t)i;
     } else if (!(i & 1ull) && !(j[0] && !j[1] && !j[-1])) {
-      pk[i >> 1] = 0xFFFFFFFF00000000ull | (uint32_t)mix64(i);
+      pk[i >> 1] = pair_hole_word((uint32_t)mix64(i));
       pv[i >> 1] = EMPTY;
     }
     if (i == 0) *np = nfixed;
@@ -805,20 +814,45 @@
   B.pv = w7 + P.pv, B.ftable = w7 + P.ftable, B.fbits = w7 + P.fbits;
   if (nf) {
     ELP_HIP(c, hipMemsetAsync(B.ftable, 0xFF, Tf * sizeof(uint32_t), st));
-    ELP_LAUNCH(c, "md_frag_insert", k_frag_insert, dim3(blocks_for(nf, 256)), dim3(256), 0, B.m, (const uint4 *)B.fkey, (const uint32_t *)B.flist, nf, B.ftable, Tf - 1, B.rep, B.best);
+    ELP_LAUNCH(c, "md_frag_insert", k_frag_insert, dim3(blocks_for(nf, 256)), dim3(256), 0, (const uint4 *)B.fkey, (const uint32_t *)B.flist, nf, B.ftable, Tf - 1, B.rep);
     ELP_LAUNCH(c, "md_frag_bits", k_frag_bits, dim3(blocks_for(Tf / 32, 256)), dim3(256), 0, (const uint32_t *)B.ftable, Tf / 32, B.fbits);
   }
   const auto front = fuse_adapt ? k_md_front<true> : k_md_front<false>;
-  ELP_LAUNCH(c, "md_front", front, dim3(S.front_grid), dim3(MF_THREADS), 0, fc, (const int32_t *)c->score.p, c->upos.p, c->key.p, B.fkey, B.code, B.hash32, B.hash_lo, B.bloom,
+  ELP_LAUNCH(c, "md_front", front, dim3(S.front_grid), dim3(MF_THREADS), 0, fc, c->upos.p, c->key.p, B.fkey, B.code, B.hash32, B.hash_lo, B.bloom,
              (uint32_t)(S.bw - 1), B.n_table_dev, (const uint32_t *)B.ftable, (const uint32_t *)B.fbits, nf ? Tf - 1 : (uint64_t)0, B.best, c->mate.p, c->pair_win.p, B.pk, B.pv, B.np_dev, S.nfx,
              c->tune.mate_path == 0 ? 1 : 0);
   return 0;
 }
 
-static int md_fragments(elp_ctx *c, const MdBufs &B, uint32_t nf, uint32_t *n_tab_out) {
+struct ScoreLane {
+  elp_ctx *c;
+  bool open = false, pending = false;
+  explicit ScoreLane(elp_ctx *ctx) : c(ctx) {}
+  ScoreLane(const ScoreLane &) = delete;
+  ScoreLane &operator=(const ScoreLane &) = delete;
+  int begin() {
+    open = true;
+    return adapt_scores_beside(c, &pending);
+  }
+  int join() {
+    if (!open) return 0;
+    open = false;
+    ELP_TRY(score_lane_join(c));
+    c->derived.scores = true;
+    c->derived.adapt_pending = pending;
+    return 0;
+  }
+  ~ScoreLane() {
+    if (open && c->score_done) (void)hipStreamWaitEvent(c->stream, c->score_done, 0);
+  }
+};
+
+static int md_fragments(elp_ctx *c, const MdBufs &B, ScoreLane &lane, uint32_t nf, uint32_t *n_tab_out) {
   hipStream_t st = c->stream;
+  ELP_TRY(lane.join());
   if (nf) {
     const unsigned fgrid = blocks_for(nf, 256);
+    ELP_LAUNCH(c, "md_frag_best", k_frag_best, dim3(fgrid), dim3(256), 0, (const int32_t *)c->score.p, (const uint32_t *)B.flist, nf, (const uint32_t *)B.rep, B.best);
     ELP_LAUNCH(c, "md_frag_tie", k_frag_tie, dim3(fgrid), dim3(256), 0, B.m, (const uint32_t *)B.flist, nf, (const uint32_t *)B.rep, (const unsigned long long *)B.best, B.winner);
     ELP_LAUNCH(c, "md_frag_flag", k_frag_flag, dim3(fgrid), dim3(256), 0, B.m, (const uint32_t *)B.flist, nf, (const uint32_t *)B.rep, (const unsigned long long *)B.best,
                (const uint32_t *)B.winner, c->flag.p);
@@ -925,13 +959,19 @@
   ELP_TRY(md_carve(c, L, &B));
   const FrontCols fc{n, c->refid.p, c->pos.p, c->flag.p, c->has_sr.p, c->rgid.p, c->rg_lib.p, c->split.p, c->cigar_off.p, c->cigar.p, c->qname_off.p, c->qname.p,
                      (uint32_t)c->n_ref, pos_bits};
+  ScoreLane lane(c);
+  const bool beside = fuse_adapt && c->tune.score_lane != 0;
+  if (beside) ELP_TRY(lane.begin());
   ELP_TRY(md_frag_list(c, S, B, fc));
-  if (fuse_adapt) ELP_TRY(adapt_scores(c));
+  if (fuse_adapt && !beside) ELP_TRY(adapt_scores(c));
   uint32_t nf = 0, n_tab = 0;
   ELP_TRY(md_front(c, S, L, B, fc, fuse_adapt, &nf));
-  if (fuse_adapt) c->derived.keys = c->derived.scores = true;
+  if (fuse_adapt) {
+    c->derived.keys = true;
+    if (!beside) c->derived.scores = true;
+  }
   ELP_TRY(sort_presort(c));
-  ELP_TRY(md_fragments(c, B, nf, &n_tab));
+  ELP_TRY(md_fragments(c, B, lane, nf, &n_tab));
   const MatePlan P = mate_plan(n, n_tab, c->tune.mate_path, S.T);
   bool big = false;
   if (!P.fast) ELP_TRY(md_mates(c, S, B, P, n_tab, &big));
diff --git a/elprep_amd/csrc/markdup_plan.hpp b/elprep_amd/csrc/markdup_plan.hpp
--- a/elprep_amd/csrc/markdup_plan.hpp
+++ b/elprep_amd/csrc/markdup_plan.hpp
@@ -12,6 +12,16 @@
 constexpr int PB_CAP = 1024;
 constexpr int FLI_CHUNK = 2048;
 constexpr int MF_THREADS = 320, MF_RECS = 312;
+
+constexpr int PB_ECAP = 1024;
+
+constexpr uint32_t PE_LIVE = 0u, PE_HOLE = 0xFFFFFFFFu;
+inline constexpr uint64_t pair_entry_word(uint32_t hash32) { return ((uint64_t)PE_LIVE << 32) | hash32; }
+inline constexpr uint64_t pair_hole_word(uint32_t scatter32) { return ((uint64_t)PE_HOLE << 32) | scatter32; }
+inline constexpr bool pair_word_is_hole(uint64_t pk) { return (uint32_t)(pk >> 32) == PE_HOLE; }
+inline constexpr uint32_t pair_word_hash(uint64_t pk) { return (uint32_t)pk; }
+constexpr uint32_t PB_SINGLE = 0xFFFFFFFEu;
+inline constexpr size_t pair_bucket_lds() { return (size_t)PB_CAP * (8 + 4 + 4) + (size_t)PB_ECAP * 2 + 16; }
 
 inline unsigned md_blocks(uint64_t n, unsigned per_block) { return (unsigned)((n + per_block - 1) / per_block); }
 
```

Result: no change. 2490 (median of 2 runs) (-0.2%).
